# Daniel-Lin-S/decode_tonal_langauge

Hardware: AMD Instinct MI355X
Metric: mel-frames/sec (train step) SynthesisModelCNN, 128ch x 400t batch256 (higher is better)
Workload: dtype f32; 1 GPU; SynthesisModelCNN 128ch x 400t -> 80 mel, 4 tones x 2 syllables, L=5, global batch 256 (strong scaling: 256 windows on rank 0), dropout 0.5, NAdam, 1,376,768,720 params; per_gpu_batch=256, global_batch=256, parallelism=dp1, init=drawn on every rank

## Files before the change

### decode_tonal_langauge_amd/_conv_stack.py

```python
from __future__ import annotations

from typing import List

import torch

from . import _kernels, _lib
from ._launch import LaunchTimers, launch_nt, launch_tn, permute_reduce, r4
from ._lib import (EPI_C1WGRAD, EPI_GY, EPI_LRELU, EPI_MASK, EPI_MASKY, EPI_POOL, EPI_POOLV, LOAD_DIRECT, LOAD_UNPOOL, LOAD_V,
                   LOAD_Y, check, ptr)


class _Stage:

    def __init__(self, idx, cin, cout, k, pool, tin, tp_in):
        self.idx, self.cin, self.cout, self.k, self.pool = idx, cin, cout, k, pool
        self.tin, self.tp_in = tin, tp_in
        self.tc = tin - k + 1
        self.tout = self.tc // 2 if pool else self.tc
        self.tp_out = tp_in // 2 if pool else tp_in


class ConvStack(LaunchTimers):
    F63_CAPABLE = True

    def __init__(self, n_channels: int, n_timepoints: int, stage_defs, negative_slope: float, conv_channels: int):
        if negative_slope < 0:
            raise ValueError("the MI355X path needs negative_slope >= 0 (max-pool / LeakyReLU are fused)")
        self.lib = _lib.load()
        self.C = n_channels
        self.T = n_timepoints
        self.slope = float(negative_slope)
        k1 = stage_defs[0][1]
        npool_after = sum(1 for s in stage_defs[1:] if s[2])
        tc1 = n_timepoints - k1 + 1
        self.k1 = k1
        self.c1 = stage_defs[0][0]
        self.tout1 = tc1 // 2
        if not stage_defs[0][2]:
            raise ValueError("first stage must pool")
        align = 1 << npool_after
        self.tp1 = max(align, (self.tout1 + align - 1) // align * align)
        _kernels.validate()
        self.wino63 = (self.F63_CAPABLE and _kernels.get("wino") == "6"
                       and self._f63_covers(stage_defs, n_timepoints))
        tp1_default = self.tp1
        if self.wino63:
            self.tp1 = (self.tout1 + 11) // 12 * 12
        self.f63_yprod = (self.wino63 and _kernels.get("f63_yprod") != "0" and stage_defs[0][0] % 256 == 0
                          and self.tp1 >= 12)
        self.f63_yprod3 = (self.wino63 and _kernels.get("f63_yprod") != "0" and stage_defs[1][0] % 256 == 0)
        self.stages: List[_Stage] = []
        cin, tin, tp = self.c1, self.tout1, self.tp1
        for i, (cout, k, pool) in enumerate(stage_defs[1:], start=2):
            st = _Stage(i, cin, cout, k, pool, tin, tp)
            if st.tout < 1:
                raise ValueError("n_timepoints too small for the conv stack")
            if self.wino63 and i == 3:
                st.tp_out = tp1_default // 4
            self.stages.append(st)
            cin, tin, tp = cout, st.tout, st.tp_out
        self.gy4 = self._gy_applies()
        self.lat = tin
        self.tp5 = tp
        self.ld5 = r4(conv_channels)
        mode = _kernels.get("wino")
        self.wino43 = mode != "0"
        self.store_p1 = _kernels.get("store_p1") == "1"
        self.fuse_c1 = True
        self.wino_vout = True
        self.tn_bm = 0
        self._gy_A = None
        self._vhalo = {}
        self._B = None
        self.generation = 0

    def _alloc(self, B: int, dev) -> bool:
        if self._B == B and self._dev == dev:
            return False
        self._B, self._dev = B, dev
        self.S = B * self.C
        self._v_ready = {}
        self._gy_A = None
        self._vhalo = {}
        self._alloc_rows()
        self.Yt = {}
        self._y_ready = {}
        self.V = {}
        self.Vd = {}
        self._vd_ready = {}
        self.G = None
        return True

    def _alloc_rows(self):
        S, dev = self.S, self._dev
        z = lambda *s: torch.zeros(*s, dtype=torch.float32, device=dev)
        zi = lambda *s: torch.zeros(*s, dtype=torch.int32, device=dev)
        self.P = {}
        if not (self.wino63 or self._conv1_writes_v()) or self.store_p1:
            self.P[1] = z(S * self.tp1, self.c1)
        self.bits = {1: zi(S * self.tp1, self.c1 // 32)}
        self.sbits = {1: zi(S * self.tp1, self.c1 // 32)}
        for st in self.stages:
            rows = S * st.tp_out
            ld = st.cout if st.pool else self.ld5
            no_rows = (self.wino63 and st.idx == 2) or (self._writes_v(st) and not self._f63(st))
            if not no_rows or self.store_p1:
                self.P[st.idx] = z(rows, ld)
            if st.pool:
                self.bits[st.idx] = zi(rows, st.cout // 32)
                self.sbits[st.idx] = zi(rows, st.cout // 32)

    def _alloc_bwd(self) -> bool:
        if self.G is not None:
            return False
        z = lambda *s: torch.zeros(*s, dtype=torch.float32, device=self._dev)
        S = self.S
        self.G = {}
        if not self.wino63 and not (self.fuse_c1 and self._c1_fusable() and self._v43(self.stages[0])):
            self.G[1] = z(S * self.tp1, self.c1)
        for st in self.stages:
            if not (self.f63_yprod and st.idx == 2) and not (self.gy4 and st.idx == 3):
                self.G[st.idx] = z(S * st.tp_out, st.cout if st.pool else self.ld5)
        return True

    def _stream(self):
        return torch.cuda.current_stream().cuda_stream

    def _permute(self, src, dst, dims, strides, *args, **kw):
        permute_reduce(self.lib, src, dst, dims, strides, *args, **kw)

    def _nt(self, tag=None, fn="tl_gemm_nt_window", **kw):
        ev = self._tick(tag)
        launch_nt(self.lib, fn, **kw)
        if ev:
            ev[1].record()

    def _tn(self, tag=None, fn="tl_gemm_tn_window", **kw):
        ev = self._tick(tag)
        launch_tn(self.lib, fn, **kw)
        if ev:
            ev[1].record()

    @staticmethod
    def _splitk(tiles: int, ksteps: int, target: int = 2048) -> int:
        return int(max(1, min(ksteps, (target + tiles - 1) // tiles, 1024)))

    def _tn_stored(self, tag, At, ldt, W, rows, K):
        if ldt <= 32:
            sk = self._splitk((K + 511) // 512, (rows + 15) // 16, 1024)
        else:
            sk = self._splitk(((ldt + 127) // 128) * ((K + 127) // 128), (rows + 31) // 32, 1024)
        slab = torch.empty(sk, ldt, K, dtype=torch.float32, device=self._dev)
        self._tn(tag=tag, A=ptr(At), B=ptr(W), slab=ptr(slab), Krows=rows, A_rows=rows, B_rows=rows, Mdim=ldt, Ndim=K, lda=ldt,
                 ldb=K, ldc=K, loader=LOAD_DIRECT, splitk=sk, slab_stride=ldt * K)
        return slab, sk

    def _pack_conv(self, w, cin_ld, flip_for_dgrad):
        O, I, J, _ = w.shape
        if not flip_for_dgrad:
            dst = torch.empty(J, O, cin_ld, dtype=torch.float32, device=w.device)
            self._permute(w, dst, (1, J, O, cin_ld), (0, 1, I * J, J), (1, J, O, I))
            return dst
        old = r4(O)
        dst = torch.empty(J, cin_ld, old, dtype=torch.float32, device=w.device)
        self._permute(w, dst, (1, J, cin_ld, old), (0, -1, J, I * J), (1, J, I, O), src_off=J - 1)
        return dst

    @staticmethod
    def _f63_covers(stage_defs, T) -> bool:
        if len(stage_defs) < 4:
            return False
        (c1, k1, p1), (c2, k2, p2), (c3, k3, p3) = stage_defs[0], stage_defs[1], stage_defs[2]
        tout1 = (T - k1 + 1) // 2
        tout2 = (tout1 - 2) // 2
        tout3 = (tout2 - 2) // 2
        return (p1 and p2 and p3 and k2 == 3 and k3 == 3 and 1 <= k1 <= 3 and c1 in (128, 256, 512, 1024)
                and c2 % 128 == 0 and c3 % 64 == 0 and tout3 >= 1 and T >= 2 * tout1 + 2)

    def _f63(self, st) -> bool:
        return self.wino63 and st.idx in (2, 3)

    def _nt63_rows(self) -> int:
        return int(self.lib.tl_wino63_nt_tile_rows())

    def _v_hex_buffer(self, store, idx, rows, cin):
        nh = rows // 6
        nh_pad = (nh + 24 + 127) // 128 * 128
        V = store.get(idx)
        if V is None or V.shape[0] != nh_pad or V.shape[1] != 8 or V.shape[2] != cin:
            V = store[idx] = torch.zeros(nh_pad, 8, cin, dtype=torch.float32, device=self._dev)
        return V

    def _halo_buffer(self, key, ntm, cout):
        halo = self._vhalo.get(key)
        if halo is None or halo.shape[0] != ntm or halo.shape[2] != cout:
            halo = self._vhalo[key] = torch.zeros(ntm, 2, cout, dtype=torch.float32, device=self._dev)
        return halo

    def _pack_wino63(self, w, forward: bool):
        O, I = w.shape[0], w.shape[1]
        dst = torch.empty(8, O, I, dtype=torch.float32, device=w.device) if forward else \
            torch.empty(8, I, O, dtype=torch.float32, device=w.device)
        check(self.lib.tl_wino63_weights(ptr(w), ptr(dst) if forward else None, None if forward else ptr(dst), O, I, I, O,
                                         self._stream()), "tl_wino63_weights")
        return dst

    def f63_issue_factor(self, st) -> float:
        return (st.tp_in // 6) * 8.0 / (st.tc * 3.0)

    def _stage_forward63(self, st, w, bia) -> None:
        S = self.S
        wp = self._pack_wino63(w, True)
        V = self._v_ready[st.idx - 1]
        if st.idx == 2 and self.store_p1 and 2 not in self.P:
            self.P[2] = torch.zeros(S * st.tp_out, st.cout, dtype=torch.float32, device=self._dev)
        Pout = self.P.get(st.idx) if (st.idx != 2 or self.store_p1) else None
        kw = dict(A=ptr(V), A_rows=V.shape[0], lda=V.shape[2], loader=LOAD_V, Bw=ptr(wp), bias=ptr(bia), out=ptr(Pout),
                  M=S * st.tp_in, N=st.cout, K=st.cin, ldb=st.cin, ldo=Pout.shape[1] if Pout is not None else st.cout, J=3,
                  row_shift=0, Tp=st.tp_in, slope=self.slope, obits=ptr(self.bits[st.idx]), osign=ptr(self.sbits[st.idx]),
                  ld_obits=st.cout // 32, Tvalid=2 * st.tout)
        if st.idx == 2:
            rows_out = S * st.tp_out
            Vn = self._v_hex_buffer(self.V, 2, rows_out, st.cout)
            ntm = -(-(S * st.tp_in) // self._nt63_rows())
            halo = self._halo_buffer(2, ntm, st.cout)
            kw.update(epilogue=EPI_POOLV, vout=ptr(Vn), vhalo=ptr(halo), vout_quads=Vn.shape[0], ld_vout=Vn.shape[2])
            self._nt(tag="conv2_fwd", fn="tl_conv3_wino63v_nt", **kw)
            check(self.lib.tl_wino63_v_fixup(ptr(Vn), ptr(halo), rows_out // 6, ntm, st.tp_out, st.cout, Vn.shape[2],
                                             self._stream()), "tl_wino63_v_fixup")
            self._v_ready[2] = Vn
        else:
            if Pout is None:
                raise RuntimeError("F(6,3) stage 3 writes pooled rows: its output buffer was not allocated")
            kw.update(epilogue=EPI_POOL, out_tp=st.tp_out)
            self._nt(tag="conv3_fwd", fn="tl_conv3_wino63v_nt", **kw)

    def _stage_wgrad63(self, st, gw, gb) -> None:
        S = self.S
        f32 = dict(dtype=torch.float32, device=self._dev)
        rows_in = S * st.tp_in
        nd = st.cout
        ldg = nd
        V = self._v_ready[st.idx - 1]
        tiles = (st.cin // 64) * (nd // 64)
        sk = self._splitk(tiles, (rows_in + 35) // 36, 4096)
        slab = torch.empty(sk, 8 * st.cin, ldg, **f32)
        bias_part = torch.empty(sk, nd, **f32)
        if (st.idx == 3 and self.f63_yprod3 and self._y_ready.get(3) != self.generation):
            Gs = self.G[3]
            Y3 = self._v_hex_buffer(self.Yt, 3, rows_in, nd)
            Vd3 = self._v_hex_buffer(self.Vd, 3, rows_in, nd)
            ev = self._tick("conv3_yvd")
            check(self.lib.tl_wino63_unpool_yvd(ptr(Gs), ptr(self.bits[3]), ptr(Y3), ptr(Vd3), rows_in, Gs.shape[0], st.tp_in,
                                                st.tp_out, 2 * st.tout, nd, Gs.shape[1], st.cout // 32, nd, self._stream()),
                  "tl_wino63_unpool_yvd")
            if ev:
                ev[1].record()
            self._y_ready[3] = self.generation
            self._vd_ready[3] = self.generation
        if self._y_ready.get(st.idx) == self.generation:
            Y = self.Yt[st.idx]
            self._y_ready[st.idx] = -1
            self._tn(tag=f"conv{st.idx}_wgrad", fn="tl_conv3_wino63v_tn", A=ptr(V), B=ptr(Y), slab=ptr(slab), Krows=rows_in,
                     A_rows=V.shape[0], B_rows=Y.shape[0], Mdim=st.cin, Ndim=nd, lda=V.shape[2], ldb=Y.shape[2], ldc=ldg, J=3,
                     Tp=st.tp_in, splitk=sk, slab_stride=8 * st.cin * ldg, loader=LOAD_Y, Tvalid=2 * st.tout,
                     colsum=ptr(bias_part))
        else:
            Gs = self.G[st.idx]
            Vd = self._v_hex_buffer(self.Vd, st.idx, rows_in, nd)
            self._tn(tag=f"conv{st.idx}_wgrad", fn="tl_conv3_wino63v_tn", A=ptr(V), B=ptr(Gs), slab=ptr(slab), Krows=rows_in,
                     A_rows=V.shape[0], B_rows=Gs.shape[0], Mdim=st.cin, Ndim=nd, lda=V.shape[2], ldb=Gs.shape[1], ldc=ldg, J=3,
                     Tp=st.tp_in, splitk=sk, slab_stride=8 * st.cin * ldg, loader=LOAD_UNPOOL, bbits=ptr(self.bits[st.idx]),
                     ld_bbits=st.cout // 32, Tvalid=2 * st.tout, colsum=ptr(bias_part), vd=ptr(Vd), ld_vd=nd, g_tp=st.tp_out)
            self._vd_ready[st.idx] = self.generation
        self._wino_wgrad_tail(st, slab, bias_part, 8, "tl_wino63_wgrad_finalize", gw, gb)

    def _wino_wgrad_tail(self, st, slab, bias_part, taps, finalize, gw, gb) -> None:
        sk, rows, ldg = slab.shape
        if sk > 1:
            red = torch.empty(rows, ldg, dtype=torch.float32, device=self._dev)
            n = taps * st.cin * ldg
            self._permute(slab, red, (1, 1, 1, n), (0, 0, 0, 1), nz=sk, zs=n)
        else:
            red = slab
        check(getattr(self.lib, finalize)(ptr(red), ptr(gw), st.cout, st.cin, ldg, self._stream()), finalize)
        self._permute(bias_part, gb, (1, 1, 1, st.cout), (0, 0, 0, 1), nz=sk, zs=bias_part.shape[1])

    def _gy_stage(self, st) -> bool:
        return self.gy4 and st.idx == 4

    def _gy_applies(self) -> bool:
        if not (self.wino63 and self.f63_yprod3 and len(self.stages) >= 3):
            return False
        below, st = self.stages[1], self.stages[2]
        return (_kernels.get("conv4_dgrad") == "nt63" and st.k == 1 and st.pool and self._f63(below)
                and st.cout % 32 == 0 and st.cout >= 40 and st.cin % 32 == 0 and (below.tp_in // 2) % 3 == 0)

    def _stage_dgrad_gy(self, st, w):
        S = self.S
        below = self.stages[1]
        tpg = below.tp_in // 2
        rows = S * tpg
        f32 = dict(dtype=torch.float32, device=self._dev)
        nh = -(-rows // 6)
        nh_pad = (nh + 127) // 128 * 128
        A = self._gy_A
        if A is None or A.shape[0] != nh_pad or A.shape[2] != st.cout:
            A = self._gy_A = torch.zeros(nh_pad, 8, st.cout, **f32)
        Gs = self.G[st.idx]
        ev = self._tick(f"conv{st.idx}_dgrad")
        check(self.lib.tl_wino63_unpool_rows6(ptr(Gs), ptr(self.bits[st.idx]), ptr(A), rows, Gs.shape[0], tpg, st.tp_out,
                                              2 * st.tout, st.cout, Gs.shape[1], st.cout // 32, st.cout, 0, self._stream()),
              "tl_wino63_unpool_rows6")
        taps = torch.empty(st.cout // 8, 8, st.cin, 8, **f32)
        check(self.lib.tl_wino63_weights1(ptr(w), ptr(taps), st.cout, st.cin, st.cout, self._stream()), "tl_wino63_weights1")
        rows3 = S * below.tp_in
        Y3 = self._v_hex_buffer(self.Yt, below.idx, rows3, below.cout)
        Vd3 = self._v_hex_buffer(self.Vd, below.idx, rows3, below.cout)
        ntm = -(-rows // self._nt63_rows())
        halo = self._halo_buffer("d3", ntm, below.cout)
        self._nt(tag=None, fn="tl_conv1_wino63v_dgrad_nt", A=ptr(A), A_rows=A.shape[0], lda=A.shape[2], loader=LOAD_V,
                 Bw=ptr(taps), M=rows, N=st.cin, K=st.cout, ldb=st.cout, ldo=st.cin, J=1, row_shift=0, Tp=tpg, slope=self.slope,
                 auxbits=ptr(self.sbits[below.idx]), ld_auxbits=self.sbits[below.idx].shape[1], abits=ptr(self.bits[below.idx]),
                 ld_abits=below.cout // 32, out_tp=below.tp_out, Tvalid_in=2 * below.tout, epilogue=EPI_GY, out=None,
                 vout=ptr(Y3), vout2=ptr(Vd3), vhalo=ptr(halo), vout_quads=Y3.shape[0], ld_vout=Y3.shape[2])
        check(self.lib.tl_wino63_vd_fixup(ptr(Vd3), ptr(halo), rows // 3, ntm, below.tp_in // 6, below.cout, Vd3.shape[2],
                                          self._stream()), "tl_wino63_vd_fixup")
        if ev:
            ev[1].record()
        self._y_ready[below.idx] = self.generation
        self._vd_ready[below.idx] = self.generation
        return None

    def _stage_dgrad63(self, st, w):
        S = self.S
        rows_in = S * st.tp_in
        if self._vd_ready.get(st.idx) != self.generation:
            raise RuntimeError("F(6,3) input gradient: its operand (Vd from the stage's weight-gradient pass, or Y2 from the "
                               "input gradient of stage 3) must be written first")
        self._vd_ready[st.idx] = -1
        on_y = st.idx == 2 and self.f63_yprod
        Vd = self.Yt[2] if on_y else self.Vd[st.idx]
        if on_y:
            wd = torch.empty(8, st.cin, st.cout, dtype=torch.float32, device=w.device)
            check(self.lib.tl_wino63_weights_y(ptr(w), ptr(wd), st.cout, st.cin, st.cout, self._stream()), "tl_wino63_weights_y")
        else:
            wd = self._pack_wino63(w, False)
        kw = dict(A=ptr(Vd), A_rows=Vd.shape[0], lda=Vd.shape[2], loader=LOAD_V, Bw=ptr(wd), M=rows_in, N=st.cin,
                  K=st.cout, ldb=st.cout, ldo=st.cin, J=3, row_shift=0 if on_y else -2, Tp=st.tp_in, slope=self.slope,
                  auxbits=ptr(self.sbits[st.idx - 1]), ld_auxbits=self.sbits[st.idx - 1].shape[1])
        if st.idx == 3 and self.f63_yprod:
            below = self.stages[0]
            rows2 = S * below.tp_in
            Y2 = self._v_hex_buffer(self.Yt, 2, rows2, below.cout)
            Vd2 = self._v_hex_buffer(self.Vd, 2, rows2, below.cout) if self.store_p1 else None
            ntm = -(-rows_in // self._nt63_rows())
            halo = self._halo_buffer("d2", ntm, below.cout) if self.store_p1 else None
            self._nt(tag="conv3_dgrad", fn="tl_conv3_wino63v_nt", epilogue=EPI_MASKY, out=None, vout=ptr(Y2), vout2=ptr(Vd2),
                     vhalo=ptr(halo), vout_quads=Y2.shape[0], ld_vout=Y2.shape[2], abits=ptr(self.bits[2]),
                     ld_abits=below.cout // 32, Tvalid_in=2 * below.tout, **kw)
            if Vd2 is not None:
                check(self.lib.tl_wino63_vd_fixup(ptr(Vd2), ptr(halo), rows_in // 3, ntm, below.tp_in // 6, below.cout,
                                                  Vd2.shape[2], self._stream()), "tl_wino63_vd_fixup")
            self._y_ready[2] = self.generation
            self._vd_ready[2] = self.generation
            return None
        if st.idx == 3:
            self._nt(tag="conv3_dgrad", fn="tl_conv3_wino63v_nt", epilogue=EPI_MASK, out=ptr(self.G[2]), **kw)
            return None
        ntm = -(-rows_in // self._nt63_rows())
        part = torch.empty(ntm, (self.k1 + 1) * self.c1, dtype=torch.float32, device=self._dev)
        self._nt(tag="conv2_dgrad", fn="tl_conv3_wino63v_nt", epilogue=EPI_C1WGRAD, out=None, c1x=ptr(self._x),
                 c1bits=ptr(self.bits[1]), c1partial=ptr(part), c1T=self.T, c1kt=self.k1, Tvalid=self.tout1, **kw)
        return part

    def _c1_fusable(self) -> bool:
        return self.k1 <= 3 and self.T >= 2 * self.tout1 + 2

    def _v43(self, st) -> bool:
        return (self.wino43 and st.k == 3 and st.pool and st.cin % 64 == 0 and st.cout % 32 == 0 and st.tp_in % 4 == 0
                and r4(st.cout) % 16 == 0)

    def _tn_bm(self, st) -> int:
        wide = st.cin % 128 == 0
        dma8 = wide and r4(st.cout) % 64 == 0 and (st.cout // 32) % 2 == 0
        if self.tn_bm == 127:
            return 127 if wide else 64
        if self.tn_bm in (0, 128):
            return 128 if dma8 else 64
        return 64

    def _conv1_writes_v(self) -> bool:
        return (self._v43(self.stages[0]) and self.tp1 % 4 == 0 and self.c1 in (128, 256, 512, 1024)
                and (self.fuse_c1 and self._c1_fusable()))

    def _writes_v(self, st) -> bool:
        if not (self.wino_vout and st.pool and st.idx - 1 < len(self.stages)):
            return False
        nxt = self.stages[st.idx - 1]
        return self._v43(st) and self._v43(nxt) and st.tp_in % 8 == 0 and nxt.cin == st.cout

    def _pin(self, st):
        return self.P.get(st.idx - 1)

    def _v_buffer(self, idx, rows, cin, store=None):
        store = self.V if store is None else store
        nq = rows // 4
        nq_pad = (nq + 127) // 128 * 128
        V = store.get(idx)
        if V is None or V.shape[0] != nq_pad or V.shape[2] != cin:
            V = store[idx] = torch.zeros(nq_pad, 6, cin, dtype=torch.float32, device=self._dev)
        return V

    def _input_transform(self, st):
        src = self.P[st.idx - 1]
        V = self._v_buffer(st.idx - 1, src.shape[0], st.cin)
        ev = self._tick(f"conv{st.idx}_xform")
        check(self.lib.tl_wino43_input_transform(ptr(src), ptr(V), src.shape[0], st.tp_in, st.cin, src.shape[1], st.cin,
                                                 self._stream()), "tl_wino43_input_transform")
        if ev:
            ev[1].record()
        return V

    def wgrad_issue_factor(self, st) -> float:
        if self._f63(st):
            return self.f63_issue_factor(st)
        return 0.5 if self._v43(st) else 1.0

    def kernel_families(self):
        if self.wino63:
            self._fam_share = {}
            st2, st3 = self.stages[0], self.stages[1]
            f6 = "Winograd F(6,3) on pre-transformed operands, LDS-DMA"
            tn = "wino63v_tn4_kernel<true>" if st3.cin % 256 == 0 and st3.tp_in >= 12 else "wino63v_tn_kernel<true>"
            tn2 = "wino63v_tn4_kernel<true>" if st2.cin % 256 == 0 else "wino63v_tn_kernel<true>"
            fams = {f"wino63v_nt_kernel<POOLV> (conv2 forward, {f6}; writes V of its pooled output for conv3)": ["conv2_fwd"],
                    f"wino63v_nt_kernel<POOL> (conv3 forward, {f6})": ["conv3_fwd"],
                    f"wino63v_nt_kernel<C1WGRAD> (conv2 input gradient + conv1 weight gradient, {f6})": ["conv2_dgrad"],
                    }
            if self.f63_yprod3:
                gy = self.gy4
                src = "the epilogue of conv4's input gradient" if gy else "wino63_unpool_yvd_kernel"
                fams[f"wino63v_tn4y_kernel (conv3 weight gradient, {f6}: both operands by LDS-DMA, no transform in the kernel; Y3 / Vd3 "
                     f"from {src})"] = ["conv3_wgrad"]
            else:
                fams[f"{tn} (conv3 weight gradient, {f6}; also writes Vd)"] = ["conv3_wgrad"]
            if self.f63_yprod:
                both = "Y and Vd" if self.store_p1 else "Y"
                fams[f"wino63v_nt_kernel<MASKY> (conv3 input gradient, {f6}; writes {both} of conv2 instead of the gradient rows)"] = ["conv3_dgrad"]
                fams[f"wino63v_tn4y_kernel (conv2 weight gradient, {f6}: both operands by LDS-DMA, no transform in the kernel)"] = ["conv2_wgrad"]
            else:
                fams[f"wino63v_nt_kernel<MASK> (conv3 input gradient, {f6})"] = ["conv3_dgrad"]
                fams[f"{tn2} (conv2 weight gradient, {f6}; also writes Vd)"] = ["conv2_wgrad"]
            issued = {k: self.f63_issue_factor(st2 if "conv2" in k else st3) for k in fams}
            return fams, issued
        self._fam_share = {}
        if not all(self._v43(st) for st in self.stages[:2]):
            fams = {"nt_window_kernel<128,UNPOOL,MASK> (conv input-gradient)": ["conv2_dgrad", "conv3_dgrad", "conv4_dgrad"],
                    "nt_window_kernel<128,DIRECT,POOL> (conv forward)": ["conv2_fwd", "conv3_fwd", "conv4_fwd"],
                    "tn3_kernel<UNPOOL> (conv weight-gradient)": ["conv2_wgrad", "conv3_wgrad"]}
            return fams, {k: 1.0 for k in fams}
        form = "Winograd F(4,3) on pre-transformed operands, LDS-DMA"
        fused = self.fuse_c1 and self._c1_fusable()
        bm = self._tn_bm(self.stages[0])
        extra = {}
        if bm == 128:
            tn = f"wino43v_tn8_kernel<true> (conv2/conv3 weight gradient, {form}; also writes Vd for the input gradient)"
        else:
            ntm = (self.stages[0].cin + 63) // 64
            tn = f"wino43v_tn_kernel<false, 2> (conv2/conv3 weight gradient, C_in tiles 1..{ntm - 1} of {ntm}, {form})"
            vdn = f"wino43v_tn_kernel<true, 2> (conv2/conv3 weight gradient, C_in tile 0 of {ntm}, {form}, + writes Vd for the input gradient)"
            extra[vdn] = ["conv2_wgrad_vd", "conv3_wgrad_vd"]
            self._fam_share = {tn: (ntm - 1) / ntm, vdn: 1.0 / ntm}
        fams = {tn: ["conv2_wgrad", "conv3_wgrad"]}
        if self._writes_v(self.stages[0]):
            fams[f"wino43v_nt_kernel<POOLV> (conv2 forward, {form}; writes V of its pooled output for conv3 instead of the raw rows)"] = ["conv2_fwd"]
            fams[f"wino43v_nt_kernel<POOL> (conv3 forward, {form})"] = ["conv3_fwd"]
        else:
            fams[f"wino43v_nt_kernel<POOL> (conv2/conv3 forward, {form})"] = ["conv2_fwd", "conv3_fwd"]
        fams.update(extra)
        if fused:
            fams[f"wino43v_nt_kernel<UNPOOL,C1WGRAD> (conv2 input gradient + conv1 weight gradient, {form})"] = ["conv2_dgrad"]
            fams[f"wino43v_nt_kernel<UNPOOL,MASK> (conv3 input gradient, {form})"] = ["conv3_dgrad"]
        else:
            fams[f"wino43v_nt_kernel<UNPOOL,MASK> (conv2/conv3 input gradient, {form})"] = ["conv2_dgrad", "conv3_dgrad"]
        return fams, {k: 0.5 for k in fams}

    def _pack_wino43(self, w, forward: bool):
        O, I = w.shape[0], w.shape[1]
        dst = torch.empty(6, O, I, dtype=torch.float32, device=w.device) if forward else \
            torch.empty(6, I, O, dtype=torch.float32, device=w.device)
        check(self.lib.tl_wino43_weights(ptr(w), ptr(dst) if forward else None, None if forward else ptr(dst), O, I, I, O,
                                         self._stream()), "tl_wino43_weights")
        return dst

    def conv1_forward(self, x, w1, b1) -> None:
        lib, st_ = self.lib, self._stream()
        S, T, dev = self.S, self.T, self._dev
        self._x = x
        self._v_ready = {}
        w1 = w1.reshape(self.c1, self.k1).contiguous()
        sbits = ptr(self.sbits.get(1))
        if self.store_p1 and 1 not in self.P:
            self.P[1] = torch.zeros(S * self.tp1, self.c1, dtype=torch.float32, device=dev)
        P1 = ptr(self.P[1]) if self.store_p1 else None
        geom = (S, T, self.k1, self.c1, self.tp1, self.tout1, self.slope, st_)
        if self.wino63:
            V1 = self._v_hex_buffer(self.V, 1, S * self.tp1, self.c1)
            ev = self._tick("conv1_fwd")
            check(lib.tl_conv1_fwd_v6(ptr(x), ptr(w1), ptr(b1), P1, ptr(V1), ptr(self.bits[1]), sbits, *geom), "tl_conv1_fwd_v6")
            if ev:
                ev[1].record()
            self._v_ready[1] = V1
        elif self._conv1_writes_v():
            V1 = self._v_buffer(1, S * self.tp1, self.c1)
            check(lib.tl_conv1_fwd_v(ptr(x), ptr(w1), ptr(b1), P1, ptr(V1), ptr(self.bits[1]), sbits, *geom), "tl_conv1_fwd_v")
            self._v_ready[1] = V1
        else:
            check(lib.tl_conv1_fwd(ptr(x), ptr(w1), ptr(b1), ptr(self.P[1]), ptr(self.bits[1]), sbits, *geom), "tl_conv1_fwd")

    STAGE_NAMES = {2: "ecog_conv_block.3", 3: "ecog_conv_block.6", 4: "ecog_conv_block.9", 5: "ecog_conv_block.12"}

    def stage_forward(self, st: _Stage, w: torch.Tensor, bia: torch.Tensor) -> None:
        if self._f63(st):
            return self._stage_forward63(st, w, bia)
        S = self.S
        v43 = self._v43(st)
        wp = self._pack_wino43(w, True) if v43 else self._pack_conv(w, st.cin, False)
        src = self._pin(st)
        vout = self._writes_v(st)
        if vout and self.store_p1 and st.idx not in self.P:
            self.P[st.idx] = torch.zeros(S * st.tp_out, st.cout, dtype=torch.float32, device=self._dev)
        Pout = self.P.get(st.idx) if (not vout or self.store_p1) else None
        kw = dict(A=ptr(src), Bw=ptr(wp), bias=ptr(bia), out=ptr(Pout), M=S * st.tp_in,
                  A_rows=S * st.tp_in, N=st.cout, K=st.cin, lda=st.cin, ldb=st.cin,
                  ldo=Pout.shape[1] if Pout is not None else st.cout, J=st.k, row_shift=0, Tp=st.tp_in, slope=self.slope,
                  loader=LOAD_DIRECT)
        if st.pool:
            kw.update(epilogue=EPI_POOL, obits=ptr(self.bits[st.idx]), osign=ptr(self.sbits[st.idx]),
                      ld_obits=st.cout // 32, Tvalid=2 * st.tout)
        else:
            kw.update(epilogue=EPI_LRELU, Tvalid=st.tout)
        if not v43:
            self._nt(tag=f"conv{st.idx}_fwd", fn="tl_gemm_nt_window", **kw)
            return
        V = self._v_ready.get(st.idx - 1)
        if V is None:
            V = self._v_ready[st.idx - 1] = self._input_transform(st)
        kw.update(A=ptr(V), A_rows=V.shape[0], lda=V.shape[2], loader=LOAD_V)
        if vout:
            rows_out = S * st.tp_out
            Vn = self._v_buffer(st.idx, rows_out, st.cout)
            ntm = (S * st.tp_in + 511) // 512
            halo = self._halo_buffer(st.idx, ntm, st.cout)
            kw.update(epilogue=EPI_POOLV, vout=ptr(Vn), vhalo=ptr(halo), vout_quads=Vn.shape[0], ld_vout=Vn.shape[2])
            self._nt(tag=f"conv{st.idx}_fwd", fn="tl_conv3_wino43v_nt", **kw)
            check(self.lib.tl_wino43_v_fixup(ptr(Vn), ptr(halo), rows_out // 4, ntm, st.tp_out, st.cout, Vn.shape[2],
                                             self._stream()), "tl_wino43_v_fixup")
            self._v_ready[st.idx] = Vn
            return
        self._nt(tag=f"conv{st.idx}_fwd", fn="tl_conv3_wino43v_nt", **kw)

    def _colsum(self, Gm, rows, ncols, ld, Tp, Tvalid, dst):
        nc4 = r4(ncols)
        rpb = max(1, 256 // (nc4 // 4))
        nblk = int(min(2048, max(1, rows // (rpb * 16))))
        part = torch.empty(nblk, nc4, dtype=torch.float32, device=Gm.device)
        check(self.lib.tl_colsum(ptr(Gm), ptr(part), nblk, rows, nc4, ld, Tp, Tvalid, self._stream()), "tl_colsum")
        self._permute(part, dst, (1, 1, 1, ncols), (0, 0, 0, 1), nz=nblk, zs=nc4)

    def _reduce_c1_partials(self, part: torch.Tensor, gw: torch.Tensor, gb: torch.Tensor) -> None:
        f32 = dict(dtype=torch.float32, device=part.device)
        nblk = part.shape[0]
        zs = (self.k1 + 1) * self.c1
        if nblk >= 256 and zs % 4 == 0:
            red = torch.empty(zs, **f32)
            flat = part.view(-1)
            for c0 in range(0, zs, 1024):
                nc = min(1024, zs - c0)
                self._colsum(flat[c0:], nblk, nc, zs, 1, 1, red[c0:c0 + nc])
            self._permute(red, gw, (1, 1, self.c1, self.k1), (0, 0, 1, self.c1))
            self._permute(red, gb, (1, 1, 1, self.c1), (0, 0, 0, 1), src_off=self.k1 * self.c1)
        else:
            self._permute(part, gw, (1, 1, self.c1, self.k1), (0, 0, 1, self.c1), nz=nblk, zs=zs)
            self._permute(part, gb, (1, 1, 1, self.c1), (0, 0, 0, 1), nz=nblk, zs=zs, src_off=self.k1 * self.c1)

    def stage_wgrad(self, st: _Stage, gw: torch.Tensor, gb: torch.Tensor) -> None:
        if self._f63(st):
            return self._stage_wgrad63(st, gw, gb)
        S = self.S
        f32 = dict(dtype=torch.float32, device=self._dev)
        Xin = self._pin(st)
        Gs = self.G[st.idx]
        rows_in = S * st.tp_in
        ldg = Gs.shape[1]
        nd = r4(st.cout)
        if self._v43(st):
            tiles = ((st.cin + 63) // 64) * ((nd + 63) // 64)
            bm = self._tn_bm(st)
            sk = self._splitk(tiles, (rows_in + 31) // 32, 4096 if bm in (127, 128) else 8192)
            slab = torch.empty(sk, 6 * st.cin, ldg, **f32)
            bias_part = torch.empty(sk, nd, **f32)
# ... 87 lines not shown
```

### decode_tonal_langauge_amd/_kernels.py

```python
from __future__ import annotations

import os
from typing import Callable, Dict, Tuple, Union

_Allowed = Union[frozenset, Callable[[str], bool]]


def _int(lo: int, hi: int) -> Callable[[str], bool]:
    def ok(v: str) -> bool:
        try:
            return lo <= int(v) <= hi
        except ValueError:
            return False
    return ok


_B = frozenset({"0", "1"})
KEYS: Dict[str, Tuple[str, _Allowed, str, str]] = {
    "wino": ("TONAL_WINO", frozenset({"6", "4", "0"}), "6",
             "conv2 / conv3: 6 Winograd F(6,3) on pre-transformed operands (F(4,3) V form where the stack does not allow it), "
             "4 the F(4,3) V form, 0 direct MFMA kernels (also the fallback for every shape neither form covers)"),
    "f63_yprod": ("TONAL_F63_YPROD", _B, "1", "F(6,3): the backward operands of stages 2 and 3 (Y2 for both passes of stage 2; Y3 / Vd3) come "
                                              "pre-transformed out of the input-gradient epilogue of the stage above (0: the weight-gradient "
                                              "kernels un-pool and transform the gradient rows themselves and write Vd)"),
    "conv4_dgrad": ("TONAL_CONV4_DGRAD", frozenset({"nt63", "gemm"}), "nt63",
                    "F(6,3): the one-tap stage behind conv3 - nt63: its input gradient on the NT63 kernel, writing Y3 / Vd3 "
                    "(no gradient rows, no tl_wino63_unpool_yvd); gemm: one-tap GEMM + tl_wino63_unpool_yvd"),
    "store_p1": ("TONAL_STORE_P1", _B, "0", "keep the raw pooled rows of stages 1 / 2 beside V, and Vd2 beside Y2 (tests)"),
    "conv7": ("TONAL_CONV7", frozenset({"wino63", "wino63bwd", "direct"}), "wino63",
              "the CNN-RNN classifier's 7-tap convolutions: wino63 three F(6,3) segments forward, direct kernels backward; "
              "wino63bwd the same forward and, in training, both backward passes on F(6,3) as well; direct all direct"),
    "whh_dh": ("TONAL_WHH_DH", _B, "1", "single process: the W_hh NAdam pass also produces the last BPTT product dh_1 = dgates_2 . W_hh "
                                        "(0: a W_hh stream of its own for it)"),
    "whh_stream": ("TONAL_WHH_STREAM", _B, "1", "label LSTM backward: dgates . W_hh as a pure stream of the weight (tl_lstm_gw; 0: the skinny "
                                                "MFMA GEMM with split-K slabs, also the form for more than 8 distinct label rows)"),
    "graph": ("TONAL_GRAPH", _B, "1", "SynthesisLite step replayed as a HIP graph"),
    "lstm_shard": ("TONAL_LSTM_SHARD", _B, "1", "data parallel: label LSTM sharded by gate rows"),
    "hilbert": ("TONAL_HILBERT", frozenset({"auto", "ols", "ols_full", "sym", "taps", "fft"}), "auto",
                "Hilbert bank: force a path (ols band-limited overlap-save, ols_full all 1024 bins per band, sym / taps the "
                "time-domain kernels with / without Hermitian symmetry, fft the DFT-domain form)"),
    "hilbert_f32": ("TONAL_HILBERT_F32", _B, "0", "float32 recordings: fp32 transforms end to end (default: fp64 math)"),
    "butter": ("TONAL_BUTTER", frozenset({"seq", "scan"}), "seq",
               "zero-phase Butterworth: seq the sequential recurrence (bit-identical to scipy's loop), scan the time-parallel "
               "block scan (2e-8 - 5e-8 from it: the size of the reference's own rounding; ~20 x faster)"),
}
_LEGACY = {v[0]: k for k, v in KEYS.items()}
_cache: Tuple[str, Dict[str, str]] = ("", {})


def _check(key: str, value: str) -> str:
    allowed = KEYS[key][1]
    ok = allowed(value) if callable(allowed) else value in allowed
    if not ok:
        what = "an integer in range" if callable(allowed) else "one of " + ", ".join(sorted(allowed))
        raise ValueError(f"TONAL_KERNELS: {key}={value!r} is not a value this switch takes ({what})")
    return value


def _parsed() -> Dict[str, str]:
    global _cache
    raw = os.environ.get("TONAL_KERNELS", "")
    if raw == _cache[0]:
        return _cache[1]
    out: Dict[str, str] = {}
    for item in raw.split(","):
        item = item.strip()
        if not item:
            continue
        key, sep, value = item.partition("=")
        key, value = key.strip(), value.strip()
        if not sep or key not in KEYS:
            raise ValueError(f"TONAL_KERNELS: unknown setting {item!r}; keys: " + ", ".join(sorted(KEYS)))
        out[key] = _check(key, value)
    _cache = (raw, out)
    return out


def get(key: str, default: str = None) -> str:
    legacy, _allowed, table_default, _doc = KEYS[key]
    spec = _parsed()
    if key in spec:
        return spec[key]
    if legacy in os.environ:
        if os.environ.get("TONAL_AB") != "1":
            raise RuntimeError(f"{legacy} is an A/B switch of the test suite and is ignored by the product: use "
                               f"TONAL_KERNELS={key}={os.environ[legacy]} (or set TONAL_AB=1 to run an A/B comparison)")
        return _check(key, os.environ[legacy])
    return table_default if default is None else default


def conv7_forward() -> str:
    form = get("conv7")
    return "wino63" if form == "wino63bwd" else form


def validate() -> None:
    _parsed()
    if os.environ.get("TONAL_AB") != "1":
        for legacy, key in _LEGACY.items():
            if legacy in os.environ:
                get(key)
```

### decode_tonal_langauge_amd/csrc/tonal_wino63.hip

```cpp
#include "tonal_common.h"
#include "tonal_wino43_epi.h"
#include "tonal_wino43v_epi.h"
#include "tonal_wino63_epi.h"
#include "tonal_wino63_kloop.h"
#include <type_traits>

namespace tl {

typedef __attribute__((address_space(3))) void lds_void6_t;
__device__ __forceinline__ void dma16h(__amdgpu_buffer_rsrc_t rs, char* lds_dst, unsigned voff, unsigned soff) {
  __builtin_amdgcn_raw_ptr_buffer_load_lds(rs, (lds_void6_t*)lds_dst, 16, voff, soff, 0, 0);
}

typedef int v6_i32x4 __attribute__((ext_vector_type(4)));
__device__ __forceinline__ v6_i32x4 v6_rsrc_words(const void* base, long long bytes) {
  const unsigned long long a = (unsigned long long)base;
  const long long n = bytes < 0 ? 0 : (bytes < 0x7fffffffLL ? bytes : 0x7fffffffLL);
  return v6_i32x4{(int)(unsigned)a, (int)(unsigned)((a >> 32) & 0xffffu), (int)n, 0x00020000};
}

__device__ __forceinline__ long long v6_at(long long hex, int i, int c, int kc8) {
  return ((((hex >> 1) * kc8 + (c >> 3)) * 8 + i) * 2 + (hex & 1)) * 8 + (c & 7);
}

// ... 48 lines not shown
  for (int t = 0; t < 8; ++t) m[t] = s[t * plane];
  const float a12 = m[1] + m[2], s12 = m[1] - m[2], a34 = m[3] + m[4], s34 = m[3] - m[4], a56 = m[5] + m[6], s56 = m[5] - m[6];
  float* d = gw + ((long long)o * I + i) * 3;
  d[0] = -m[0] - (2.f / 9.f) * a12 + (1.f / 90.f) * a34 + (32.f / 45.f) * a56;
  d[1] = -(2.f / 9.f) * s12 + (1.f / 45.f) * s34 + (16.f / 45.f) * s56;
  d[2] = -(2.f / 9.f) * a12 + (2.f / 45.f) * a34 + (8.f / 45.f) * a56 + m[7];
}

__global__ void wino63_weights7_kernel(const float* __restrict__ w, float* __restrict__ fwd, int O, int I, int taps) {
  const long long idx = (long long)blockIdx.x * blockDim.x + threadIdx.x;
  if (idx >= 3LL * O * I) return;
  const int k = (int)(idx % (3LL * I)), o = (int)(idx / (3LL * I));
  const int seg = k / I, i = k - seg * I;
  const float* s = w + ((long long)o * I + i) * taps + 3 * seg;
  const float g0 = 3 * seg < taps ? s[0] : 0.f, g1 = 3 * seg + 1 < taps ? s[1] : 0.f, g2 = 3 * seg + 2 < taps ? s[2] : 0.f;
  float* d0 = fwd + (((long long)(k >> 3) * 8) * O + o) * 8 + (k & 7);
  const long long n = (long long)O * 8;
  const float sm = g0 + g2;
  d0[0] = -g0;
  d0[n] = (-2.f / 9.f) * (sm + g1);
  d0[2 * n] = (-2.f / 9.f) * (sm - g1);
  const float a = fmaf(4.f, g2, g0), b = 2.f * g1;
  d0[3 * n] = (1.f / 90.f) * (a + b);
  d0[4 * n] = (1.f / 90.f) * (a - b);
  const float c = fmaf(4.f, g0, g2), d = 2.f * g1;
  d0[5 * n] = (8.f / 45.f) * (c + d);
  d0[6 * n] = (8.f / 45.f) * (c - d);
  d0[7 * n] = g2;
}

__global__ __launch_bounds__(256, 4) void wino63_xform2_kernel(const float* __restrict__ P, float* __restrict__ V0, float* __restrict__ V1,
                                                             long long nhex, int hps, int Tp, int Tvalid, int C, int ldp, int ldv,
                                                             int shift) {
  const int tpp = C >> 1;
  const long long idx = (long long)blockIdx.x * blockDim.x + threadIdx.x;
  const long long pair = idx / tpp;
  const int tl_ = (int)(idx - pair * tpp);
  const int half = tl_ & 1, hpar = (tl_ >> 1) & 1, kc = tl_ >> 2;
  const int c = 8 * kc + 4 * half;
  const long long hg = 2 * pair + hpar;
  if (hg >= nhex) return;
  const long long seq = hg / hps;
  const int hs = (int)(hg - seq * hps);
  const float* src = P + (seq * Tp + 6LL * hs) * (long long)ldp + c;
  f32x4 d[11];
#pragma unroll
  for (int j = 0; j < 11; ++j) {
    d[j] = f32x4{0.f, 0.f, 0.f, 0.f};
    const int t = 6 * hs + j - shift;
    if (t >= 0 && t < Tvalid) d[j] = *reinterpret_cast<const f32x4*>(src + (long long)(j - shift) * ldp);
  }
  f32x4 o0[8], o1[8];
#pragma unroll
  for (int k = 0; k < 4; ++k) {
    float a[8], b[8], va[8], vb[8];
#pragma unroll
    for (int j = 0; j < 8; ++j) {
      a[j] = d[j][k];
      b[j] = d[j + 3][k];
    }
    wino63_bt(a, va);
    wino63_bt(b, vb);
#pragma unroll
    for (int j = 0; j < 8; ++j) {
      o0[j][k] = va[j];
      o1[j][k] = vb[j];
    }
  }
  const long long at = v6_at(hg, 0, c, ldv >> 3);
#pragma unroll
  for (int j = 0; j < 8; ++j) *reinterpret_cast<f32x4*>(V0 + at + 16 * j) = o0[j];
#pragma unroll
  for (int j = 0; j < 8; ++j) *reinterpret_cast<f32x4*>(V1 + at + 16 * j) = o1[j];
}

__global__ __launch_bounds__(256, 4) void wino63_ydz_kernel(const float* __restrict__ G, float* __restrict__ Y, long long nhex, int hps,
                                                          int Tp, int Tvalid, int C, int ldg, int ldv) {
  const int tpp = C >> 1;
  const long long idx = (long long)blockIdx.x * blockDim.x + threadIdx.x;
  const long long pair = idx / tpp;
  const int tl_ = (int)(idx - pair * tpp);
  const int half = tl_ & 1, hpar = (tl_ >> 1) & 1, kc = tl_ >> 2;
  const int c = 8 * kc + 4 * half;
  const long long hg = 2 * pair + hpar;
  if (hg >= nhex) return;
  const long long seq = hg / hps;
  const int hs = (int)(hg - seq * hps);
  const float* src = G + (seq * Tp + 6LL * hs) * (long long)ldg + c;
  f32x4 d[6];
#pragma unroll
  for (int j = 0; j < 6; ++j) {
    d[j] = f32x4{0.f, 0.f, 0.f, 0.f};
    if (6 * hs + j < Tvalid) d[j] = *reinterpret_cast<const f32x4*>(src + (long long)j * ldg);
  }
  f32x4 oy[8];
#pragma unroll
  for (int k = 0; k < 4; ++k) {
    const float d6[6] = {d[0][k], d[1][k], d[2][k], d[3][k], d[4][k], d[5][k]};
    const float ev1 = (d6[0] + d6[2]) + d6[4], od1 = (d6[1] + d6[3]) + d6[5];
    const float ev2 = fmaf(16.f, d6[4], fmaf(4.f, d6[2], d6[0])), od2 = fmaf(32.f, d6[5], fmaf(8.f, d6[3], 2.f * d6[1]));
    const float ev3 = fmaf(0.0625f, d6[4], fmaf(0.25f, d6[2], d6[0])), od3 = fmaf(0.03125f, d6[5], fmaf(0.125f, d6[3], 0.5f * d6[1]));
    const float y[8] = {d6[0], ev1 + od1, ev1 - od1, ev2 + od2, ev2 - od2, ev3 + od3, ev3 - od3, d6[5]};
#pragma unroll
    for (int j = 0; j < 8; ++j) oy[j][k] = y[j];
  }
  const long long at = v6_at(hg, 0, c, ldv >> 3);
#pragma unroll
  for (int j = 0; j < 8; ++j) *reinterpret_cast<f32x4*>(Y + at + 16 * j) = oy[j];
}

__global__ __launch_bounds__(256, 4) void wino63_v_fixup_kernel(float* __restrict__ V, const float* __restrict__ halo, long long hexes,
                                                              long long tiles, int Tq, int C, int ldv) {
  const int c4n = C >> 2;
  const long long idx = (long long)blockIdx.x * blockDim.x + threadIdx.x;
  if (idx >= tiles * c4n) return;
  const long long t = idx / c4n;
  const int c = (int)(idx - t * c4n) * 4;
  const long long q = t * 64 + 63;
  if (q >= hexes) return;
  float* v = V + v6_at(q, 0, c, ldv >> 3);
  f32x4 d[8];
#pragma unroll
  for (int j = 0; j < 6; ++j) d[j] = *reinterpret_cast<const f32x4*>(v + 16 * j);
  const int tq = (int)((6 * q) % Tq);
  if (tq + 6 < Tq && t + 1 < tiles) {
    d[6] = *reinterpret_cast<const f32x4*>(halo + ((t + 1) * 2) * (long long)C + c);
    d[7] = *reinterpret_cast<const f32x4*>(halo + ((t + 1) * 2 + 1) * (long long)C + c);
  } else {
    d[6] = d[7] = f32x4{0.f, 0.f, 0.f, 0.f};
  }
  f32x4 o[8];
#pragma unroll
  for (int k = 0; k < 4; ++k) {
    float dd[8], vv[8];
#pragma unroll
    for (int j = 0; j < 8; ++j) dd[j] = d[j][k];
    wino63_bt(dd, vv);
#pragma unroll
    for (int j = 0; j < 8; ++j) o[j][k] = vv[j];
  }
#pragma unroll
  for (int j = 0; j < 8; ++j) *reinterpret_cast<f32x4*>(v + 16 * j) = o[j];
}

constexpr int V6_BH = 128, V6_BN = 64, V6_BK = 8;
constexpr int V6_ROWB = V6_BK * 4;
constexpr int V6_A_BYTES = 8 * V6_BH * V6_ROWB;
constexpr int V6_B_BYTES = 8 * V6_BN * V6_ROWB;
constexpr int V6_STAGE = V6_A_BYTES + V6_B_BYTES;
constexpr int V6_ROWS = 6 * V6_BH;

template <int EPI>
__global__ __launch_bounds__(512, 2) void wino63v_nt_kernel(const tl_nt_params p) {
  __shared__ __attribute__((aligned(1024))) char lds[3 * V6_STAGE + ((EPI == W_EPI_POOLV || EPI == W_EPI_MASKY || EPI == W_EPI_GY) ? 4096 : (EPI == W_EPI_C1W || EPI == W6_EPI_C1W_Y) ? 16384 : 0)];
  const int tid = threadIdx.x;
  const int lane = tid & 63;
  const int wave = __builtin_amdgcn_readfirstlane(tid >> 6);
  const int wm = wave >> 1, wn = wave & 1;
  const int lr = lane & 31, lh = lane >> 5;

  const int ntn = (p.N + V6_BN - 1) / V6_BN;
  const long long ntm = (p.M + V6_ROWS - 1) / V6_ROWS;
  const long long nwg = ntm * ntn;
  constexpr bool SEG3 = EPI == W_EPI_LRELU || EPI == W6_EPI_MASK7 || EPI == W6_EPI_MASK7F;
  constexpr bool SIX = EPI == W_EPI_GY;
  const int kseg = p.K / V6_BK;
  const int nsteps = SEG3 ? 3 * kseg : kseg;
  f32x16 acc[8];
  f32x4 faL[4], fbL[4], faH[4], fbH[4];

  const int prow = lane >> 1;
  const int src_chunk = (lane & 1) ^ ((lane >> 4) & 1);
  const v6_i32x4 rsB = v6_rsrc_words(p.Bw, (SIX && wave >= 6) ? 0 : 8LL * p.N * p.ldb * 4);
  const unsigned lds0 = (unsigned)(unsigned long long)(lds_void6_t*)lds;
  const unsigned dst_a0 = lds0 + (unsigned)(wave * V6_BH * V6_ROWB);
  const unsigned dst_b0 = lds0 + (unsigned)(V6_A_BYTES + wave * V6_BN * V6_ROWB);
  const int hex_of_row = (prow & 3) | ((prow >> 3) << 2) | (((prow >> 2) & 1) << 4);
  const int kc8 = p.lda >> 3;
  unsigned avoff[4], bv_lane[2];
#pragma unroll
  for (int t = 0; t < 4; ++t) avoff[t] = (unsigned)(v6_at(t * 32 + hex_of_row, wave, src_chunk * 4, kc8) * 4);
  unsigned avoff1[4];
#pragma unroll
  for (int t = 0; t < 4; ++t) avoff1[t] = SEG3 ? (unsigned)(v6_at(t * 32 + hex_of_row + 1, wave, src_chunk * 4, kc8) * 4) : avoff[t];
#pragma unroll
  for (int t = 0; t < 2; ++t) bv_lane[t] = (unsigned)((((long long)wave * p.N + t * 32 + prow) * 8 + src_chunk * 4) * 4);
  const unsigned b_step = (unsigned)p.N * 256u;

  struct tile_t {
    long long tm, R0;
    int n0;
    v6_i32x4 rsA, rsA1;
    unsigned bvoff[2];
  };
  const long long a_tile_bytes = (long long)V6_BH * 8 * p.lda * 4, a_total_bytes = p.A_rows * 8LL * p.lda * 4;
  auto place = [&](tile_t& t, long long tm, int tn) {
    t.tm = tm;
    t.R0 = tm * V6_ROWS;
    t.n0 = tn * V6_BN;
    const long long ab = tm * a_tile_bytes;
    t.rsA = v6_rsrc_words(reinterpret_cast<const char*>(p.A) + ab, (SIX && wave >= 6) ? 0 : a_total_bytes - ab);
    t.rsA1 = SEG3 ? v6_rsrc_words(reinterpret_cast<const char*>(p.aux) + ab, a_total_bytes - ab) : t.rsA;
    if (t.n0 + V6_BN <= p.N) {
      const unsigned nb4 = (unsigned)t.n0 * 32u;
#pragma unroll
      for (int k = 0; k < 2; ++k) t.bvoff[k] = bv_lane[k] + nb4;
    } else {
#pragma unroll
      for (int k = 0; k < 2; ++k) {
        int n = t.n0 + k * 32 + prow;
        if (n > p.N - 1) n = p.N - 1;
        t.bvoff[k] = (unsigned)((((long long)wave * p.N + n) * 8 + src_chunk * 4) * 4);
      }
    }
  };
  tile_t cur;
  {
    long long bid = blockIdx.x;
    const long long q = nwg / 8, r = nwg % 8, x = bid % 8, i = bid / 8;
    bid = (x < r ? x * (q + 1) : r * (q + 1) + (x - r) * q) + i;
    place(cur, bid / ntn, (int)(bid % ntn));
  }
  const int walk = (int)(gridDim.x >> 3), walk_q = walk / ntn, walk_r = walk - walk_q * ntn;
  auto advance = [&](const tile_t& c) -> tile_t {
    tile_t t = c;
    int tn = c.n0 / V6_BN + walk_r;
    long long tm = c.tm + walk_q;
    if (tn >= ntn) {
      tn -= ntn;
      ++tm;
    }
    place(t, tm, tn);
    return t;
  };
  auto next3 = [](int s) { return s == 2 ? 0 : s + 1; };

  const int cphys = (lh ^ ((lr >> 3) & 1)) << 4;
  const unsigned a_row = lds0 + (unsigned)((wm * 32 + lr) * V6_ROWB + cphys);
  const unsigned b_row = lds0 + (unsigned)((wn * 32 + lr) * V6_ROWB + cphys);
  int stg = 0;

  struct dma_src {
    v6_i32x4 ra;
    unsigned va[4], vb[2], sa, sb;
  };
  auto src_of = [&](const tile_t& t, int step) {
    dma_src d;
    int ks = step;
    if constexpr (SEG3) {
      const int seg = (step >= kseg ? 1 : 0) + (step >= 2 * kseg ? 1 : 0);
      ks = step - seg * kseg;
#pragma unroll
      for (int k = 0; k < 4; ++k) {
        d.ra[k] = seg == 1 ? t.rsA1[k] : t.rsA[k];
        d.va[k] = seg == 2 ? avoff1[k] : avoff[k];
      }
    } else {
      d.ra = t.rsA;
#pragma unroll
      for (int k = 0; k < 4; ++k) d.va[k] = avoff[k];
    }
    d.vb[0] = t.bvoff[0];
    d.vb[1] = t.bvoff[1];
#pragma unroll
    for (int k = 0; k < 4; ++k) d.ra[k] = __builtin_amdgcn_readfirstlane(d.ra[k]);
    d.sa = (unsigned)__builtin_amdgcn_readfirstlane(ks * 512);
    d.sb = (unsigned)__builtin_amdgcn_readfirstlane((int)((unsigned)step * b_step));
    return d;
  };
#define V6K_INPUTS(src, dst, wimm)                                                                                             \
  [a] "v"(a_row + (unsigned)stg * (unsigned)V6_STAGE), [b] "v"(b_row + (unsigned)stg * (unsigned)V6_STAGE),                    \
      [va0] "v"((src).va[0]), [va1] "v"((src).va[1]), [va2] "v"((src).va[2]), [va3] "v"((src).va[3]), [vb0] "v"((src).vb[0]), \
      [vb1] "v"((src).vb[1]), [ra] "s"((src).ra), [rb] "s"(rsB), [m0a] "s"(dst_a0 + (unsigned)(dst) * (unsigned)V6_STAGE),     \
      [m0b] "s"(dst_b0 + (unsigned)(dst) * (unsigned)V6_STAGE), [sa] "s"((src).sa), [sb] "s"((src).sb), [w] "n"(wimm)
#pragma clang diagnostic ignored "-Winline-asm"
#define V6K_STMT_R(REGS, TEXT, tl_, step, dst, wimm)                                                                     \
  do {                                                                                                                   \
    const dma_src src_ = src_of(tl_, step);                                                                              \
    asm volatile(TEXT : REGS(acc, faL, fbL, faH, fbH) : V6K_INPUTS(src_, dst, wimm) : "memory", "scc", "m0");                  \
  } while (0)
#define V6K_STMT(TEXT, tl_, step, dst, wimm) V6K_STMT_R(V6K_REGS, TEXT, tl_, step, dst, wimm)
  auto issue = [&](const tile_t& tl_, int step, int dst) {
    const dma_src src_ = src_of(tl_, step);
    asm volatile(V6K_ISSUE : : V6K_INPUTS(src_, dst, 0) : "memory", "scc", "m0");
  };
  constexpr bool early = EPI == W_EPI_POOLV || EPI == W_EPI_C1W || EPI == W6_EPI_C1W_Y;
  constexpr int NST = v6_stores<EPI>();
  constexpr int first_n = NST + 6 > 63 ? 63 : NST + 6;
  constexpr int first_wait = (first_n & 15) | (7 << 4) | (0 << 8) | ((first_n >> 4) << 14);

  issue(cur, 0, 0);
  issue(cur, 1, 1);
  __builtin_amdgcn_s_waitcnt(0x0f70);
  for (long long vb = blockIdx.x; vb < nwg; vb += gridDim.x) {
    __builtin_amdgcn_s_barrier();
    asm volatile("" ::: "memory");
    auto prefetch = [&] {
      if constexpr (EPI == W_EPI_POOL || EPI == W_EPI_POOLV || EPI == W_EPI_LRELU) return v5_prefetch_pool(p, cur.n0, wn, lr);
      else if constexpr (EPI == W_EPI_MASK || EPI == W6_EPI_MASK7) return v6_prefetch_mask(p, cur.R0, cur.n0, wm, wn, lr, lh);
      else if constexpr (EPI == W6_EPI_MASK7F) return v6_pre_mask{{0u, 0u, 0u}};
      else if constexpr (EPI == W_EPI_MASKY || EPI == W6_EPI_MASKY_Y) return v6_prefetch_masky(p, cur.R0, cur.n0, wm, wn, lr, lh);
      else if constexpr (EPI == W_EPI_GY) return v6_prefetch_masky<true>(p, cur.R0, cur.n0, wm, wn, lr, lh);
      else return v6_prefetch_c1w(p, cur.R0, cur.n0, wm, wn, lr, lh);
    };
    decltype(prefetch()) pre;
#define V6K_RUN(KIND, RSFX, tl_, step, dst, wimm)                                                                              \
  do {                                                                                                                         \
    if constexpr (SIX) V6K_STMT_R(V6K6_REGS##RSFX, V6K6_##KIND##_L, tl_, step, dst, wimm);                                     \
    else if constexpr (early) V6K_STMT_R(V6K_REGS##RSFX, V6K_##KIND##_E, tl_, step, dst, wimm);                                \
    else V6K_STMT_R(V6K_REGS##RSFX, V6K_##KIND##_L, tl_, step, dst, wimm);                                                     \
  } while (0)
    if constexpr (SIX) V6K_STMT_R(V6K6_REGS_FIRST, V6K6_FIRST, cur, 2, stg == 0 ? 2 : stg - 1, first_wait);
    else V6K_STMT_R(V6K_REGS_FIRST, V6K_FIRST, cur, 2, stg == 0 ? 2 : stg - 1, first_wait);
    stg = next3(stg);
    V6K_RUN(STEP1, _STEP1, cur, 3, stg == 0 ? 2 : stg - 1, 0);
    stg = next3(stg);
    {
      int s = 2;
      do {
        V6K_RUN(NORM, , cur, s + 2, stg == 0 ? 2 : stg - 1, 0);
        stg = next3(stg);
      } while (++s + 2 < nsteps);
    }
    V6K_RUN(PRELAST, , cur, 0, 0, 0);
    stg = next3(stg);
    pre = prefetch();
    V6K_RUN(LAST, , cur, 0, 0, 0);
    stg = next3(stg);
#undef V6K_RUN

    const tile_t done = cur;
    const long long nb = vb + gridDim.x;
    const int last_stage = stg == 0 ? 2 : stg - 1;
    __builtin_amdgcn_s_waitcnt(0x0f70);
    if (nb < nwg) {
      cur = advance(cur);
      issue(cur, 0, stg);
      issue(cur, 1, next3(stg));
    }
    __builtin_amdgcn_sched_barrier(0);
    float* scratch = reinterpret_cast<float*>(lds + last_stage * V6_STAGE);
    (void)scratch;
    const bool full = done.R0 + V6_ROWS <= p.M && done.n0 + V6_BN <= p.N;
    if constexpr (EPI == W_EPI_POOL) {
      if (full) v6_epilogue_pool<false, true>(p, acc, pre, nullptr, done.R0, done.n0, wm, wn, lr, lh, done.tm);
      else v6_epilogue_pool<false, false>(p, acc, pre, nullptr, done.R0, done.n0, wm, wn, lr, lh, done.tm);
    } else if constexpr (EPI == W_EPI_POOLV) {
      float* xch = reinterpret_cast<float*>(lds + 3 * V6_STAGE);
      if (full) v6_epilogue_pool<true, true>(p, acc, pre, xch, done.R0, done.n0, wm, wn, lr, lh, done.tm);
      else v6_epilogue_pool<true, false>(p, acc, pre, xch, done.R0, done.n0, wm, wn, lr, lh, done.tm);
    } else if constexpr (EPI == W_EPI_LRELU) {
      if (full) v6_epilogue_lrelu<true>(p, acc, pre, done.R0, done.n0, wm, wn, lr, lh);
      else v6_epilogue_lrelu<false>(p, acc, pre, done.R0, done.n0, wm, wn, lr, lh);
    } else if constexpr (EPI == W_EPI_MASK || EPI == W6_EPI_MASK7) {
      if (full) v6_epilogue_mask<true>(p, acc, pre, done.R0, done.n0, wm, wn, lr, lh);
      else v6_epilogue_mask<false>(p, acc, pre, done.R0, done.n0, wm, wn, lr, lh);
    } else if constexpr (EPI == W6_EPI_MASK7F) {
      if (full) v6_epilogue_mask<true, true>(p, acc, pre, done.R0, done.n0, wm, wn, lr, lh);
      else v6_epilogue_mask<false, true>(p, acc, pre, done.R0, done.n0, wm, wn, lr, lh);
    } else if constexpr (EPI == W_EPI_MASKY) {
      float* xch = reinterpret_cast<float*>(lds + 3 * V6_STAGE);
      if (full) v6_epilogue_masky<true>(p, acc, pre, xch, done.R0, done.n0, wm, wn, lr, lh, done.tm);
      else v6_epilogue_masky<false>(p, acc, pre, xch, done.R0, done.n0, wm, wn, lr, lh, done.tm);
    } else if constexpr (EPI == W6_EPI_MASKY_Y) {
      if (full) v6_epilogue_masky<true, false, false>(p, acc, pre, nullptr, done.R0, done.n0, wm, wn, lr, lh, done.tm);
      else v6_epilogue_masky<false, false, false>(p, acc, pre, nullptr, done.R0, done.n0, wm, wn, lr, lh, done.tm);
    } else if constexpr (EPI == W_EPI_GY) {
      float* xch = reinterpret_cast<float*>(lds + 3 * V6_STAGE);
      if (full) v6_epilogue_masky<true, true>(p, acc, pre, xch, done.R0, done.n0, wm, wn, lr, lh, done.tm);
      else v6_epilogue_masky<false, true>(p, acc, pre, xch, done.R0, done.n0, wm, wn, lr, lh, done.tm);
    } else {
      v6_epilogue_c1w<EPI == W6_EPI_C1W_Y>(p, acc, pre, reinterpret_cast<float*>(lds + 3 * V6_STAGE) + wave * 512, scratch, done.R0,
                                           done.n0, wm, wn, lr, lh, done.tm);
    }
    {
      constexpr int n = NST + 6 > 63 ? 63 : NST + 6;
      __builtin_amdgcn_s_waitcnt((n & 15) | (7 << 4) | (15 << 8) | ((n >> 4) << 14));
    }
  }
}



constexpr int T6_BN = 64, T6_H = 6;
constexpr int T6_PLANE = T6_H * 64;
constexpr int T6_TILE = 8 * T6_PLANE;
constexpr int T6_NA = 4, T6_NG = 6;
constexpr int T6_GW = T6_H * 4 * 64;
constexpr int T6_GT = T6_GW + 64;

template <bool WVD>
__global__ __launch_bounds__(512, 1) void wino63v_tn_kernel(const tl_tn_params p, int mtn) {
  constexpr int NA = T6_NA, NG = T6_NG, GW = T6_GW, GT = T6_GT;
  __shared__ __attribute__((aligned(1024))) float lds[(NA * 2 + 2) * T6_TILE + NG * GT];
  float* As = lds;
  float* Bs = lds + NA * 2 * T6_TILE;
  float* Gs = Bs + 2 * T6_TILE;
  const int tid = threadIdx.x, lane = tid & 63;
  const int wave = __builtin_amdgcn_readfirstlane(tid >> 6);
  const int wm = wave >> 1, wn = wave & 1, lr = lane & 31, lh = lane >> 5;
  const int ntn = p.Ndim / T6_BN;
  const long long tiles = (long long)mtn * ntn;
  const long long nwg = tiles * p.splitk;
  long long bid = (long long)blockIdx.y * gridDim.x + blockIdx.x;
  {
    const long long q = nwg / 8, r = nwg % 8, x = bid % 8, i = bid / 8;
    bid = (x < r ? x * (q + 1) : r * (q + 1) + (x - r) * q) + i;
  }
  const int z = __builtin_amdgcn_readfirstlane((int)(bid / tiles));
  const int tt = __builtin_amdgcn_readfirstlane((int)(bid % tiles));
  const int mi = __builtin_amdgcn_readfirstlane(tt / ntn);
  const int m0 = mi * 128, n0 = __builtin_amdgcn_readfirstlane((tt % ntn) * T6_BN);

  const long long hexes_all = p.Krows / 6;
  const long long ksteps_all = (hexes_all + T6_H - 1) / T6_H;
  const long long per = __builtin_amdgcn_readfirstlane((int)((ksteps_all + p.splitk - 1) / p.splitk));
  const long long ks_begin = z * per;
  long long ks_end = ks_begin + per;
  if (ks_end > ksteps_all) ks_end = ksteps_all;
  const int nsteps = ks_end > ks_begin ? (int)(ks_end - ks_begin) : 0;

  f32x16 acc[8];
#pragma unroll
  for (int i = 0; i < 8; ++i)
#pragma unroll
    for (int e = 0; e < 16; ++e) acc[i][e] = 0.f;

  const long long v_h0 = ks_begin * T6_H;
  const int kc8 = p.lda >> 3;
  const __amdgpu_buffer_rsrc_t rsV = __builtin_amdgcn_make_buffer_rsrc(
      (void*)(p.A + v_h0 * 8 * (long long)p.lda), 0, clip31((p.A_rows - v_h0) * 8 * (long long)p.lda * 4), 0x00020000);
  unsigned vvoff[3], vdst[3];
#pragma unroll
  for (int t = 0; t < 3; ++t) {
    const int half = (wave * 3 + t) / 12, pc = (wave * 3 + t) % 12;
    const int rho = 4 * pc + (lane >> 4), i = rho / 6, hx = rho % 6;
    const int chunk = (lane & 15) ^ ((hx & 1) << 3);
    vvoff[t] = (unsigned)(v6_at(hx, i, m0 + half * 64 + chunk * 4, kc8) * 4);
    vdst[t] = (unsigned)((half * T6_TILE + pc * 256) * 4);
  }
  const unsigned v_step = (unsigned)(T6_H * 8 * p.lda * 4);
  auto issue_v = [&](int step) {
    char* base = reinterpret_cast<char*>(As) + (step & (NA - 1)) * (2 * T6_TILE * 4);
    const unsigned soff = (unsigned)step * v_step;
#pragma unroll
    for (int t = 0; t < 3; ++t) dma16h(rsV, base + vdst[t], vvoff[t] + soff, 0u);
  };
  const int Tq = p.Tp >> 1, hps = p.Tp / 6;
  const int g_tp = p.g_tp > 0 ? p.g_tp : Tq;
  const bool wpiece = wave >= 6;
  const int myhex = wpiece ? (lane >> 3) : wave;
  const long long seq0 = v_h0 / hps;
  const int hs0 = (int)(v_h0 - seq0 * hps);
  const long long g_r0 = seq0 * g_tp + 3LL * hs0;
  int g_hs = hs0 + myhex, g_off = 3 * myhex;
  while (g_hs >= hps) {
    g_hs -= hps;
    g_off += g_tp - Tq;
  }
  const int ldw4 = p.ld_bbits * 4;
  const __amdgpu_buffer_rsrc_t rsG = __builtin_amdgcn_make_buffer_rsrc(
      wpiece ? (void*)(p.bbits + g_r0 * (long long)p.ld_bbits + (n0 >> 5)) : (void*)(p.B + g_r0 * (long long)p.ldb + n0), 0,
      wpiece ? clip31((p.B_rows - g_r0) * (long long)ldw4 - (long long)(n0 >> 5) * 4)
             : clip31((p.B_rows - g_r0) * (long long)p.ldb * 4 - (long long)n0 * 4),
      0x00020000);
  const unsigned g_lane = wpiece ? (unsigned)(((lane >> 1) & 3) * ldw4 + (lane & 1) * 4)
                                 : (unsigned)(((lane >> 4) * (long long)p.ldb + (lane & 15) * 4) * 4);
  const unsigned g_row4 = wpiece ? (unsigned)ldw4 : (unsigned)(p.ldb * 4);
  const unsigned gdst = wpiece ? (unsigned)(GW * 4) : (unsigned)(wave * 256 * 4);
  const bool g_live = !wpiece || lane < 48;
  auto issue_g = [&](int slot) {
    const unsigned voff = g_live ? (unsigned)g_off * g_row4 + g_lane : 0xfffffff0u;
    if (wpiece) __builtin_amdgcn_raw_ptr_buffer_load_lds(rsG, (lds_void6_t*)(reinterpret_cast<char*>(Gs) + slot * (GT * 4) + gdst), 4, voff, 0u, 0, 0);
    else dma16h(rsG, reinterpret_cast<char*>(Gs) + slot * (GT * 4) + gdst, voff, 0u);
    g_hs += T6_H;
    g_off += 3 * T6_H;
    while (g_hs >= hps) {
      g_hs -= hps;
      g_off += g_tp - Tq;
    }
  };
  auto next6 = [](int v) { return v == NG - 1 ? 0 : v + 1; };

  constexpr bool write_vd = WVD;
  const bool ywave = wave < T6_H;
  const int sw = lane ^ ((wave & 1) << 5);
  int tq = __builtin_amdgcn_readfirstlane((int)((6 * (v_h0 + (ywave ? wave : 0))) % p.Tp));
  const int dstep = __builtin_amdgcn_readfirstlane((6 * T6_H) % p.Tp);
  float bsum = 0.f;
  const int kcd = write_vd ? (p.ld_vd >> 3) : 1;
  const unsigned vd_pstride = (unsigned)(16 * p.ld_vd * 4);
  const long long vd_hexes = ((hexes_all + 1) >> 1) << 1;
  const __amdgpu_buffer_rsrc_t rsVd = __builtin_amdgcn_make_buffer_rsrc(
      write_vd ? (void*)(p.vd + v_h0 * 8 * (long long)p.ld_vd) : (void*)p.slab, 0,
      write_vd ? clip31((vd_hexes - v_h0) * 8 * (long long)p.ld_vd * 4) : 0, 0x00020000);
  const unsigned vdA_lane = (unsigned)(v6_at(0, lane & 3, n0 + (lane & ~3), kcd) * 4);
  const unsigned vdB_lane = vdA_lane + 4u * 64u;
  const int nhex = (int)hexes_all, h_first = (int)v_h0;
  const int h_end = h_first + nsteps * T6_H;
  const int hs_lim = nhex < h_end ? nhex : h_end;
  struct y_in {
    float g[3];
    unsigned long long mo[3], me[3];
    int tq;
  };
  struct y_out {
    float d[6];
  };
  auto uni = [](unsigned long long v) -> unsigned long long {
    return (unsigned long long)(unsigned)__builtin_amdgcn_readfirstlane((int)(unsigned)v) |
           ((unsigned long long)(unsigned)__builtin_amdgcn_readfirstlane((int)(unsigned)(v >> 32)) << 32);
  };
  const int wy = ywave ? wave : 0;
  auto fetch_y = [&](int sd, int slot, y_in& y) {
    const int h = h_first + sd * T6_H + wy;
    const int live = ywave & (h < hs_lim);
    const float* gs = Gs + slot * GT;
    const unsigned long long* ws = reinterpret_cast<const unsigned long long*>(gs + GW) + wy * 4;
#pragma unroll
    for (int r = 0; r < 3; ++r) {
      y.g[r] = gs[wy * 256 + r * 64 + lane];
      const unsigned long long w = uni(ws[r]);
      const int v = live & (tq + 2 * r < p.Tvalid);
// ... 444 lines not shown
  };
#pragma unroll
  for (int i = 0; i < 8; ++i) fac[i] = 0.f;
#pragma unroll
  for (int i = 0; i < 4; ++i) fbc[i] = 0.f;

  {
    issue_v(0);
    issue_v(1);
    issue_v(2);
    issue_g(0);
    issue_g(1);
    issue_g(2);
    issue_g(3);
    float gp0 = 0.f;
    unsigned long long wp0 = 0ull;
    if (write_vd && hs0 > 0) {
      const long long pr = g_r0 - 1;
      if (pr < p.B_rows) {
        gp0 = p.B[pr * (long long)p.ldb + n0 + lane];
        const uint32_t* wsrc = p.bbits + pr * (long long)p.ld_bbits + (n0 >> 5);
        wp0 = (unsigned long long)wsrc[0] | ((unsigned long long)wsrc[1] << 32);
      }
    }
    __builtin_amdgcn_s_waitcnt(0x0070);
    __builtin_amdgcn_s_barrier();
    asm volatile("" ::: "memory");
    {
      y_in y0;
      fetch_y(0, 0, y0);
      const y_out u0 = compute_y(0, y0);
      if (write_vd && mi == 0) {
        float gp;
        unsigned long long wp;
        front_row(0, NG - 1, gp, wp);
        if (wave == 0) {
          gp = gp0;
          wp = uni(wp0);
        }
        vd_part(0, y0.tq, u0, gp, wp);
      }
    }
    __builtin_amdgcn_s_waitcnt(0x0070);
    __builtin_amdgcn_s_barrier();
    asm volatile("" ::: "memory");
  }
  int slot1 = 1, slot4 = 4;
  int turn = 1;
  for (int s = 0; s < nsteps; ++s) {
    const int abuf = s & (NA - 1), bbuf = s & 1;
    const int slot0 = slot1 == 0 ? NG - 1 : slot1 - 1;
    __builtin_amdgcn_sched_barrier(0);
    issue_v(s + 3);
    issue_g(slot4);
    y_raw yr;
    fetch_raw(slot1, yr);
    load_frag(fa0, fb0, abuf, bbuf, 0);
    mfma8(fac, fbc);
    load_frag(fa1, fb1, abuf, bbuf, 1);
    mfma8(fa0, fb0);
    __builtin_amdgcn_sched_group_barrier(0x100, 6 + 6, 0);
#pragma unroll
    for (int t = 0; t < 16; ++t) {
      __builtin_amdgcn_sched_group_barrier(0x008, 1, 0);
      if (t < 4) __builtin_amdgcn_sched_group_barrier(0x010, 1, 0);
      if (t >= 4 && t < 10) __builtin_amdgcn_sched_group_barrier(0x100, 1, 0);
    }
    __builtin_amdgcn_sched_barrier(0);
    load_frag(fac, fbc, abuf, bbuf, 2);
    y_in yn;
    y_out un = {};
    masks_y(s + 1, yr, yn);
    un = compute_y(s + 1, yn);
    mfma8(fa1, fb1);
    __builtin_amdgcn_sched_group_barrier(0x100, 6, 0);
#pragma unroll
    for (int t = 0; t < 8; ++t) {
      __builtin_amdgcn_sched_group_barrier(0x008, 1, 0);
      __builtin_amdgcn_sched_group_barrier(0x002, 5, 0);
      if (t >= 6) __builtin_amdgcn_sched_group_barrier(0x200, 2, 0);
    }
    __builtin_amdgcn_sched_barrier(0);
    if constexpr (write_vd) {
      if (ywave && turn == mi && s + 1 < nsteps) {
        float gp;
        unsigned long long wp;
        front_row(slot1, slot0, gp, wp);
        vd_part(s + 1, yn.tq, un, gp, wp);
      }
      turn = turn + 1 == nslots ? 0 : turn + 1;
    }
    __builtin_amdgcn_s_waitcnt(0x0078);
    __builtin_amdgcn_s_barrier();
    asm volatile("" ::: "memory");
    slot1 = next6(slot1);
    slot4 = next6(slot4);
  }
  mfma8(fac, fbc);

  if (p.colsum != nullptr && mi == 0) {
    __syncthreads();
    float* red = lds;
    red[wave * 64 + lane] = ywave ? bsum : 0.f;
    __syncthreads();
    if (tid < 64) {
      float t = 0.f;
#pragma unroll
      for (int q = 0; q < T6_H; ++q) t += red[q * 64 + tid];
      p.colsum[(long long)z * p.Ndim + n0 + tid] = t;
    }
  }
  float* out = p.slab + (long long)z * p.slab_stride;
  const int col = n0 + wn * 32 + lr;
#pragma unroll
  for (int i = 0; i < 8; ++i)
#pragma unroll
    for (int e = 0; e < 16; ++e) {
      const int m = m0 + wm * 64 + (i >> 2) * 32 + (e & 3) + 8 * (e >> 2) + 4 * lh;
      out[((long long)(i0 + (i & 3)) * p.Mdim + m) * (long long)p.ldc + col] = acc[i][e];
    }
}

__global__ __launch_bounds__(256, 4) void wino63_vd_fixup_kernel(float* __restrict__ Vd, const float* __restrict__ halo, long long hexes,
                                                               long long tiles, int hps, int C, int ldv) {
  const int c4n = C >> 2;
  const long long idx = (long long)blockIdx.x * blockDim.x + threadIdx.x;
  if (idx >= tiles * c4n) return;
  const long long t = idx / c4n;
  const int c = (int)(idx - t * c4n) * 4;
  const long long q = t * 256;
  if (q >= hexes) return;
  float* v = Vd + v6_at(q, 0, c, ldv >> 3);
  f32x4 d[8];
#pragma unroll
  for (int j = 2; j < 8; ++j) d[j] = *reinterpret_cast<const f32x4*>(v + 16 * j);
  if (t > 0 && (q % hps) != 0) {
    d[0] = *reinterpret_cast<const f32x4*>(halo + ((t - 1) * 2) * (long long)C + c);
    d[1] = *reinterpret_cast<const f32x4*>(halo + ((t - 1) * 2 + 1) * (long long)C + c);
  } else {
    d[0] = d[1] = f32x4{0.f, 0.f, 0.f, 0.f};
  }
  f32x4 o[8];
#pragma unroll
  for (int k = 0; k < 4; ++k) {
    float dd[8], vv[8];
#pragma unroll
    for (int j = 0; j < 8; ++j) dd[j] = d[j][k];
    wino63_bt(dd, vv);
#pragma unroll
    for (int j = 0; j < 8; ++j) o[j][k] = vv[j];
  }
#pragma unroll
  for (int j = 0; j < 8; ++j) *reinterpret_cast<f32x4*>(v + 16 * j) = o[j];
}

__global__ __launch_bounds__(512, 1) void wino63v_tn4y_kernel(const tl_tn_params p, int mtn) {
  constexpr int NA = 4;
  constexpr int QT = 4 * T6_PLANE;
  __shared__ __attribute__((aligned(1024))) float lds[NA * 4 * QT + NA * QT + 256];
  float* As = lds;
  float* Ys = lds + NA * 4 * QT;
  const int tid = threadIdx.x, lane = tid & 63;
  const int wave = __builtin_amdgcn_readfirstlane(tid >> 6);
  const int wm = wave >> 1, wn = wave & 1, lr = lane & 31, lh = lane >> 5;
  const int ntn = p.Ndim / T6_BN;
  const long long tiles = 2LL * mtn * ntn;
  const long long nwg = tiles * p.splitk;
  long long bid = (long long)blockIdx.y * gridDim.x + blockIdx.x;
  {
    const long long q = nwg / 8, r = nwg % 8, x = bid % 8, i = bid / 8;
    bid = (x < r ? x * (q + 1) : r * (q + 1) + (x - r) * q) + i;
  }
  const int z = __builtin_amdgcn_readfirstlane((int)(bid / tiles));
  const int tt = __builtin_amdgcn_readfirstlane((int)(bid % tiles));
  const int mi = __builtin_amdgcn_readfirstlane(tt % (2 * mtn));
  const int th = mi & 1, i0 = 4 * th;
  const int m0 = (mi >> 1) * 256, n0 = __builtin_amdgcn_readfirstlane((tt / (2 * mtn)) * T6_BN);
  const long long hexes_all = p.Krows / 6;
  const long long ksteps_all = (hexes_all + T6_H - 1) / T6_H;
  const long long per = __builtin_amdgcn_readfirstlane((int)((ksteps_all + p.splitk - 1) / p.splitk));
  const long long ks_begin = z * per;
  long long ks_end = ks_begin + per;
  if (ks_end > ksteps_all) ks_end = ksteps_all;
  const int nsteps = ks_end > ks_begin ? (int)(ks_end - ks_begin) : 0;

  f32x16 acc[8];
#pragma unroll
  for (int i = 0; i < 8; ++i)
#pragma unroll
    for (int e = 0; e < 16; ++e) acc[i][e] = 0.f;

  const long long v_h0 = ks_begin * T6_H;
  const int kc8 = p.lda >> 3, kcy = p.ldb >> 3;
  const __amdgpu_buffer_rsrc_t rsV = __builtin_amdgcn_make_buffer_rsrc(
      (void*)(p.A + v_h0 * 8 * (long long)p.lda), 0, clip31((p.A_rows - v_h0) * 8 * (long long)p.lda * 4), 0x00020000);
  const __amdgpu_buffer_rsrc_t rsY = __builtin_amdgcn_make_buffer_rsrc(
      (void*)(p.B + v_h0 * 8 * (long long)p.ldb), 0, clip31((p.B_rows - v_h0) * 8 * (long long)p.ldb * 4), 0x00020000);
  unsigned vvoff[3], vdst[3];
#pragma unroll
  for (int t = 0; t < 3; ++t) {
    const int quarter = (wave * 3 + t) / 6, pc = (wave * 3 + t) % 6;
    const int rho = 4 * pc + (lane >> 4), i = rho / 6, hx = rho % 6;
    const int chunk = (lane & 15) ^ ((hx & 1) << 3);
    vvoff[t] = (unsigned)(v6_at(hx + p.a_hex, i0 + i, m0 + quarter * 64 + chunk * 4, kc8) * 4);
    vdst[t] = (unsigned)((quarter * QT + pc * 256) * 4);
  }
  const bool ypiece = wave < T6_H;
  unsigned yvoff;
  {
    const int rho = 4 * (ypiece ? wave : 0) + (lane >> 4), i = rho / 6, hx = rho % 6;
    const int chunk = (lane & 15) ^ ((hx & 1) << 3);
    yvoff = (unsigned)(v6_at(hx, i0 + i, n0 + chunk * 4, kcy) * 4);
  }
  const unsigned v_step = (unsigned)(T6_H * 8 * p.lda * 4), y_step = (unsigned)(T6_H * 8 * p.ldb * 4);
  auto issue = [&](int step) {
    char* vb = reinterpret_cast<char*>(As) + (step & (NA - 1)) * (4 * QT * 4);
    const unsigned soff = (unsigned)step * v_step;
#pragma unroll
    for (int t = 0; t < 3; ++t) dma16h(rsV, vb + vdst[t], vvoff[t] + soff, 0u);
    char* yb = reinterpret_cast<char*>(Ys) + (ypiece ? ((step & (NA - 1)) * QT + wave * 256) * 4 : NA * QT * 4);
    dma16h(rsY, yb, ypiece ? yvoff + (unsigned)step * y_step : 0xfffffff0u, 0u);
  };
  const int a_off0 = wm * QT + lh * 64 + (lr ^ (lh << 5)), a_off1 = wm * QT + lh * 64 + ((32 + lr) ^ (lh << 5));
  const int b_off = lh * 64 + ((wn * 32 + lr) ^ (lh << 5));
  float fa0[8], fb0[4], fa1[8], fb1[4], fac[8], fbc[4];
  auto load_frag = [&](float (&fa)[8], float (&fb)[4], int buf, int sl) {
    const float* a_s = As + buf * (4 * QT) + sl * 128;
    const float* b_s = Ys + buf * QT + sl * 128 + b_off;
#pragma unroll
    for (int t = 0; t < 4; ++t) {
      fa[t] = a_s[a_off0 + t * T6_PLANE];
      fa[4 + t] = a_s[a_off1 + t * T6_PLANE];
      fb[t] = b_s[t * T6_PLANE];
    }
  };
  auto mfma8 = [&](const float (&fa)[8], const float (&fb)[4]) {
#pragma unroll
    for (int i = 0; i < 8; ++i) acc[i] = __builtin_amdgcn_mfma_f32_32x32x2f32(fa[i], fb[i & 3], acc[i], 0, 0, 0);
  };
#pragma unroll
  for (int i = 0; i < 8; ++i) fac[i] = 0.f;
#pragma unroll
  for (int i = 0; i < 4; ++i) fbc[i] = 0.f;
  const bool summer = p.colsum != nullptr && mi == 0 && wave == 0;
  float bsum = 0.f;
  issue(0);
  issue(1);
  issue(2);
  __builtin_amdgcn_s_waitcnt(0x0078);
  __builtin_amdgcn_s_barrier();
  asm volatile("" ::: "memory");
  for (int s = 0; s < nsteps; ++s) {
    const int buf = s & (NA - 1);
    __builtin_amdgcn_sched_barrier(0);
    issue(s + 3);
    load_frag(fa0, fb0, buf, 0);
    mfma8(fac, fbc);
    load_frag(fa1, fb1, buf, 1);
    mfma8(fa0, fb0);
    load_frag(fac, fbc, buf, 2);
    mfma8(fa1, fb1);
    __builtin_amdgcn_sched_group_barrier(0x100, 6, 0);
#pragma unroll
    for (int t = 0; t < 24; ++t) {
      __builtin_amdgcn_sched_group_barrier(0x008, 1, 0);
      if (t < 4) __builtin_amdgcn_sched_group_barrier(0x010, 1, 0);
      if (t >= 4 && t < 16) __builtin_amdgcn_sched_group_barrier(0x100, 1, 0);
    }
    __builtin_amdgcn_sched_barrier(0);
    if (summer) {
      const float* y1 = Ys + buf * QT + T6_PLANE;
#pragma unroll
      for (int hx = 0; hx < T6_H; ++hx) bsum += y1[hx * 64 + (lane ^ ((hx & 1) << 5))];
    }
    __builtin_amdgcn_s_waitcnt(0x0078);
    __builtin_amdgcn_s_barrier();
    asm volatile("" ::: "memory");
  }
  mfma8(fac, fbc);
  if (summer) p.colsum[(long long)z * p.Ndim + n0 + lane] = bsum;
  float* out = p.slab + (long long)z * p.slab_stride;
  const int col = n0 + wn * 32 + lr;
#pragma unroll
  for (int i = 0; i < 8; ++i)
#pragma unroll
    for (int e = 0; e < 16; ++e) {
      const int m = m0 + wm * 64 + (i >> 2) * 32 + (e & 3) + 8 * (e >> 2) + 4 * lh;
      out[((long long)(i0 + (i & 3)) * p.Mdim + m) * (long long)p.ldc + col] = acc[i][e];
    }
}

__global__ __launch_bounds__(256, 4) void wino63_unpool_yvd_kernel(const float* __restrict__ G, const uint32_t* __restrict__ bits,
                                                                 float* __restrict__ Y, float* __restrict__ Vd, long long nhex,
                                                                 long long g_rows, int hps, int g_tp, int Tvalid, int C, int ldg,
                                                                 int ld_bits, int ldv) {
  const int tpp = C >> 1;
  const long long idx = (long long)blockIdx.x * blockDim.x + threadIdx.x;
  const long long pair = idx / tpp;
  const int tl_ = (int)(idx - pair * tpp);
  const int half = tl_ & 1, hpar = (tl_ >> 1) & 1, kc = tl_ >> 2;
  const int c = 8 * kc + 4 * half;
  const long long hg = 2 * pair + hpar;
  if (hg >= nhex) return;
  const long long seq = hg / hps;
  const int hs = (int)(hg - seq * hps);
  const long long row0 = seq * g_tp + 3LL * hs;
// ... 257 lines not shown
  const long long n = ((nhex + 1) / 2) * (C / 2);
  TL_REQUIRE((n + 255) / 256 < (1LL << 31), "wino63_unpool_yvd: grid too large");
  hipLaunchKernelGGL(wino63_unpool_yvd_kernel, dim3((unsigned)((n + 255) / 256)), dim3(256), 0, (hipStream_t)stream, G, bits, Y, Vd,
                     nhex, (long long)g_rows, Tp / 6, g_tp, Tvalid, C, ldg, ld_bits, ldv);
  return check_launch("wino63_unpool_yvd");
}

extern "C" int tl_wino63_weights7(const float* w, float* fwd, int O, int I, int taps, void* stream) {
  using namespace tl;
  TL_REQUIRE(w && fwd && O > 0 && I > 0 && I % 8 == 0 && taps >= 7 && taps <= 9, "wino63_weights7: I %% 8 == 0 and 7..9 taps needed");
  const long long n = 3LL * O * I;
  TL_REQUIRE((n + 255) / 256 < (1LL << 31), "wino63_weights7: grid too large");
  hipLaunchKernelGGL(wino63_weights7_kernel, dim3((unsigned)((n + 255) / 256)), dim3(256), 0, (hipStream_t)stream, w, fwd, O, I, taps);
  return check_launch("wino63_weights7");
}

extern "C" int tl_wino63_xform2(const float* P, float* V0, float* V1, int64_t rows, int Tp, int Tvalid, int C, int ldp, int ldv,
                                void* stream) {
  using namespace tl;
  TL_REQUIRE(P && V0 && V1, "wino63_xform2: null pointer");
  TL_REQUIRE(Tp > 0 && Tp % 6 == 0 && rows > 0 && rows % Tp == 0 && Tvalid >= 0 && Tvalid <= Tp, "wino63_xform2: Tp %% 6 == 0, whole sequences, Tvalid <= Tp needed");
  TL_REQUIRE(C > 0 && C % 8 == 0 && ldp >= C && ldp % 4 == 0 && ldv >= C && ldv % 8 == 0, "wino63_xform2: C %% 8, ldp %% 4, ldv %% 8 needed");
  const long long nhex = rows / 6;
  const long long n = ((nhex + 1) / 2) * (C / 2);
  TL_REQUIRE((n + 255) / 256 < (1LL << 31), "wino63_xform2: grid too large");
  hipLaunchKernelGGL(wino63_xform2_kernel, dim3((unsigned)((n + 255) / 256)), dim3(256), 0, (hipStream_t)stream, P, V0, V1, nhex,
                     Tp / 6, Tp, Tvalid, C, ldp, ldv, 0);
  return check_launch("wino63_xform2");
}

extern "C" int tl_wino63_xform2s(const float* P, float* V0, float* V1, int64_t rows, int Tp, int Tvalid, int shift, int C, int ldp,
                                 int ldv, void* stream) {
  using namespace tl;
  TL_REQUIRE(P && V0 && V1, "wino63_xform2s: null pointer");
  TL_REQUIRE(Tp > 0 && Tp % 6 == 0 && rows > 0 && rows % Tp == 0 && Tvalid >= 0 && Tvalid <= Tp, "wino63_xform2s: Tp %% 6 == 0, whole sequences, Tvalid <= Tp needed");
  TL_REQUIRE(shift >= 0 && shift <= 6, "wino63_xform2s: shift must lie in 0..6");
  TL_REQUIRE(C > 0 && C % 8 == 0 && ldp >= C && ldp % 4 == 0 && ldv >= C && ldv % 8 == 0, "wino63_xform2s: C %% 8, ldp %% 4, ldv %% 8 needed");
  const long long nhex = rows / 6;
  const long long n = ((nhex + 1) / 2) * (C / 2);
  TL_REQUIRE((n + 255) / 256 < (1LL << 31), "wino63_xform2s: grid too large");
  hipLaunchKernelGGL(wino63_xform2_kernel, dim3((unsigned)((n + 255) / 256)), dim3(256), 0, (hipStream_t)stream, P, V0, V1, nhex,
                     Tp / 6, Tp, Tvalid, C, ldp, ldv, shift);
  return check_launch("wino63_xform2s");
}

extern "C" int tl_wino63_ydz(const float* G, float* Y, int64_t rows, int Tp, int Tvalid, int C, int ldg, int ldv, void* stream) {
  using namespace tl;
  TL_REQUIRE(G && Y, "wino63_ydz: null pointer");
  TL_REQUIRE(Tp > 0 && Tp % 6 == 0 && rows > 0 && rows % Tp == 0 && Tvalid >= 0 && Tvalid <= Tp, "wino63_ydz: Tp %% 6 == 0, whole sequences, Tvalid <= Tp needed");
  TL_REQUIRE(C > 0 && C % 8 == 0 && ldg >= C && ldg % 4 == 0 && ldv >= C && ldv % 8 == 0, "wino63_ydz: C %% 8, ldg %% 4, ldv %% 8 needed");
  const long long nhex = rows / 6;
  const long long n = ((nhex + 1) / 2) * (C / 2);
  TL_REQUIRE((n + 255) / 256 < (1LL << 31), "wino63_ydz: grid too large");
  hipLaunchKernelGGL(wino63_ydz_kernel, dim3((unsigned)((n + 255) / 256)), dim3(256), 0, (hipStream_t)stream, G, Y, nhex, Tp / 6, Tp,
                     Tvalid, C, ldg, ldv);
  return check_launch("wino63_ydz");
}

extern "C" int tl_conv7_wino63v_nt(const tl_nt_params* pp, void* stream) {
  using namespace tl;
  TL_REQUIRE(pp != nullptr, "conv7_wino63: null params");
  const tl_nt_params& p = *pp;
  TL_REQUIRE(p.A && p.aux && p.Bw && p.out, "conv7_wino63: null V0 (A) / V1 (aux) / Bw / out");
  TL_REQUIRE(p.loader == W_LOAD_V && p.epilogue == W_EPI_LRELU && p.row_shift == 0 && p.splitk <= 1,
             "conv7_wino63: loader 2 (pre-transformed operands), LRELU epilogue, row_shift 0, no split-K");
  TL_REQUIRE(p.J >= 7 && p.J <= 9, "conv7_wino63: 7..9 taps (three segments)");
  TL_REQUIRE(p.M > 0 && p.M % 6 == 0 && p.N > 0 && p.N % 32 == 0 && p.K >= 16 && p.K % 8 == 0, "conv7_wino63: M %% 6, N %% 32, K %% 8, K >= 16 needed");
  TL_REQUIRE(p.lda >= p.K && p.lda % 8 == 0 && p.ldb >= 3 * p.K && p.ldb % 8 == 0 && p.ldo >= p.N, "conv7_wino63: bad leading dimensions");
  TL_REQUIRE(p.A_rows % 2 == 0 && p.Tp > 0 && p.Tp % 6 == 0 && p.M % p.Tp == 0, "conv7_wino63: V holds hex pairs; Tp %% 6, whole sequences");
  TL_REQUIRE(8LL * p.N * p.ldb * 4 < (1LL << 31), "conv7_wino63: tap set larger than a buffer resource");
  TL_REQUIRE(128LL * 8 * p.lda * 4 + 4LL * p.K < (1LL << 31) && p.M + V6_ROWS < (1LL << 31), "conv7_wino63: tile span / M too large");
  TL_REQUIRE(p.slope >= 0.f && p.slope <= 1.f, "conv7_wino63: LeakyReLU slope must lie in [0, 1]");
  const long long ntm = (p.M + V6_ROWS - 1) / V6_ROWS;
  const long long nwg = ntm * ((p.N + V6_BN - 1) / V6_BN);
  TL_REQUIRE(nwg < (1LL << 31), "conv7_wino63: grid too large");
  TL_REQUIRE(p.A_rows >= ntm * V6_BH, "conv7_wino63: V0 / V1 must hold whole 128-hex tiles (pad them with zero hexes)");
  const long long ngrid = nwg < 256 ? nwg : 256;
  hipLaunchKernelGGL((wino63v_nt_kernel<W_EPI_LRELU>), dim3((unsigned)ngrid), dim3(512), 0, (hipStream_t)stream, p);
  return check_launch("conv7_wino63");
}

extern "C" int tl_conv7_wino63v_dgrad_nt(const tl_nt_params* pp, void* stream) {
  using namespace tl;
  TL_REQUIRE(pp != nullptr, "conv7_wino63_dgrad: null params");
  const tl_nt_params& p = *pp;
  TL_REQUIRE(p.A && p.aux && p.Bw && p.out, "conv7_wino63_dgrad: null V0 (A) / V1 (aux) / Bw / out");
  TL_REQUIRE(p.loader == W_LOAD_V && p.epilogue == W_EPI_MASK && p.row_shift == 0 && p.splitk <= 1,
             "conv7_wino63_dgrad: loader 2 (pre-transformed operands), MASK epilogue, row_shift 0 (the rows are moved by the transform), no split-K");
  TL_REQUIRE((p.auxbits != nullptr) != (p.mask != nullptr), "conv7_wino63_dgrad: exactly one mask source - auxbits (sign words) or mask (float rows)");
  TL_REQUIRE(p.J == 7, "conv7_wino63_dgrad: 7 taps");
  TL_REQUIRE(p.M > 0 && p.M % 6 == 0 && p.N > 0 && p.N % 32 == 0 && p.K >= 16 && p.K % 8 == 0, "conv7_wino63_dgrad: M %% 6, N %% 32, K %% 8, K >= 16 needed");
  TL_REQUIRE(p.lda >= p.K && p.lda % 8 == 0 && p.ldb >= 3 * p.K && p.ldb % 8 == 0 && p.ldo >= p.N, "conv7_wino63_dgrad: bad leading dimensions");
  TL_REQUIRE(p.auxbits == nullptr || p.ld_auxbits * 32 >= p.N, "conv7_wino63_dgrad: ld_auxbits too small");
  TL_REQUIRE(p.mask == nullptr || p.ld_mask >= p.N, "conv7_wino63_dgrad: ld_mask too small");
  TL_REQUIRE(p.A_rows % 2 == 0 && p.Tp > 0 && p.Tp % 6 == 0 && p.M % p.Tp == 0, "conv7_wino63_dgrad: V holds hex pairs; Tp %% 6, whole sequences");
  TL_REQUIRE(8LL * p.N * p.ldb * 4 < (1LL << 31), "conv7_wino63_dgrad: tap set larger than a buffer resource");
  TL_REQUIRE(128LL * 8 * p.lda * 4 + 4LL * p.K < (1LL << 31) && p.M + V6_ROWS < (1LL << 31), "conv7_wino63_dgrad: tile span / M too large");
  TL_REQUIRE(192LL * (p.ldo > p.ld_mask ? p.ldo : p.ld_mask) * 4 < (1LL << 31), "conv7_wino63_dgrad: ldo / ld_mask too large");
  TL_REQUIRE(p.slope >= 0.f && p.slope <= 1.f, "conv7_wino63_dgrad: LeakyReLU slope must lie in [0, 1]");
  const long long ntm = (p.M + V6_ROWS - 1) / V6_ROWS;
  const long long nwg = ntm * ((p.N + V6_BN - 1) / V6_BN);
  TL_REQUIRE(nwg < (1LL << 31), "conv7_wino63_dgrad: grid too large");
  TL_REQUIRE(p.A_rows >= ntm * V6_BH, "conv7_wino63_dgrad: V0 / V1 must hold whole 128-hex tiles (pad them with zero hexes)");
  const long long ngrid = nwg < 256 ? nwg : 256;
  if (p.auxbits != nullptr) hipLaunchKernelGGL((wino63v_nt_kernel<W6_EPI_MASK7>), dim3((unsigned)ngrid), dim3(512), 0, (hipStream_t)stream, p);
  else hipLaunchKernelGGL((wino63v_nt_kernel<W6_EPI_MASK7F>), dim3((unsigned)ngrid), dim3(512), 0, (hipStream_t)stream, p);
  return check_launch("conv7_wino63_dgrad");
}

extern "C" int tl_wino63_nt_tile_rows(void) { return tl::V6_ROWS; }

extern "C" int tl_conv3_wino63v_nt(const tl_nt_params* pp, void* stream) {
  using namespace tl;
  TL_REQUIRE(pp != nullptr, "wino63v_nt: null params");
  const tl_nt_params& p = *pp;
  TL_REQUIRE(p.A && p.Bw && (p.out || p.epilogue == W_EPI_C1W || p.epilogue == W_EPI_POOLV || p.epilogue == W_EPI_MASKY), "wino63v_nt: null V/Bw/out");
  TL_REQUIRE(p.loader == W_LOAD_V, "wino63v_nt: loader 2 (pre-transformed operand) only");
  TL_REQUIRE(p.J == 3 && p.splitk <= 1, "wino63v_nt: 3 taps, no split-K");
  TL_REQUIRE(p.M > 0 && p.M % 6 == 0 && p.N > 0 && p.K >= 40 && p.K % 8 == 0, "wino63v_nt: M %% 6, K %% 8, K >= 40 needed");
  TL_REQUIRE(p.lda >= p.K && p.ldb >= p.K && p.lda % 8 == 0 && p.ldb % 8 == 0, "wino63v_nt: bad leading dimensions (multiples of 8)");
  TL_REQUIRE(p.A_rows % 2 == 0, "wino63v_nt: V holds hex pairs");
  TL_REQUIRE(p.Tp > 0 && p.Tp % 6 == 0 && p.M % p.Tp == 0, "wino63v_nt: Tp must be a positive multiple of 6, M whole sequences");
  TL_REQUIRE(8LL * p.N * p.ldb * 4 < (1LL << 31), "wino63v_nt: tap set larger than a buffer resource");
  TL_REQUIRE(128LL * 8 * p.lda * 4 + 4LL * p.K < (1LL << 31), "wino63v_nt: tile span too large");
  const long long ntm = (p.M + V6_ROWS - 1) / V6_ROWS;
  const long long nwg = ntm * ((p.N + V6_BN - 1) / V6_BN);
  TL_REQUIRE(nwg < (1LL << 31), "wino63v_nt: grid too large");
  TL_REQUIRE(p.N % 32 == 0 && p.M + V6_ROWS < (1LL << 31), "wino63v_nt: N %% 32 == 0 and M < 2^31 - 768 needed");
  TL_REQUIRE(p.slope >= 0.f && p.slope <= 1.f, "wino63v_nt: LeakyReLU slope must lie in [0, 1]");
  TL_REQUIRE(p.A_rows >= ntm * V6_BH, "wino63v_nt: V must hold whole 128-hex tiles (pad it with zero hexes)");
  hipStream_t st = (hipStream_t)stream;
  const long long ngrid = nwg < 256 ? nwg : 256;
  if (p.epilogue == W_EPI_POOL) {
    TL_REQUIRE(p.row_shift == 0 && p.out && p.ldo >= p.N, "wino63v_nt: forward needs row_shift 0 and an output");
    TL_REQUIRE(p.obits != nullptr && p.Tvalid % 2 == 0 && p.Tvalid <= p.Tp, "wino63v_nt: POOL needs obits and an even Tvalid");
    TL_REQUIRE(p.ld_obits * 32 >= p.N, "wino63v_nt: POOL: ld_obits too small");
    TL_REQUIRE(p.out_tp >= 0 && (p.out_tp == 0 || 2 * p.out_tp >= p.Tvalid), "wino63v_nt: out_tp must cover the valid pooled rows");
    const long long orows = (p.M / p.Tp) * (long long)(p.out_tp > 0 ? p.out_tp : p.Tp / 2);
    TL_REQUIRE(orows * (long long)p.ldo * 4 < (1LL << 40), "wino63v_nt: output too large");
    hipLaunchKernelGGL((wino63v_nt_kernel<W_EPI_POOL>), dim3((unsigned)ngrid), dim3(512), 0, st, p);
  } else if (p.epilogue == W_EPI_POOLV) {
    TL_REQUIRE(p.row_shift == 0 && (p.out == nullptr || p.ldo >= p.N), "wino63v_nt: forward needs row_shift 0");
    TL_REQUIRE(p.obits != nullptr && p.Tvalid % 2 == 0 && p.Tvalid <= p.Tp, "wino63v_nt: POOLV needs obits and an even Tvalid");
    TL_REQUIRE(p.ld_obits * 32 >= p.N && p.Tp % 12 == 0, "wino63v_nt: POOLV needs Tp %% 12 == 0 (output hexes inside one sequence)");
    TL_REQUIRE(p.vout && p.vhalo && p.ld_vout >= p.N && p.ld_vout % 8 == 0 && p.vout_quads >= p.M / 12 && p.vout_quads % 2 == 0,
               "wino63v_nt: POOLV needs vout (>= M / 12 hexes, whole pairs, ld_vout %% 8 == 0) and vhalo");
    TL_REQUIRE(64LL * 8 * p.ld_vout * 4 < (1LL << 31), "wino63v_nt: ld_vout too large");
    hipLaunchKernelGGL((wino63v_nt_kernel<W_EPI_POOLV>), dim3((unsigned)ngrid), dim3(512), 0, st, p);
  } else if (p.epilogue == W_EPI_MASK) {
    TL_REQUIRE(p.row_shift == -2 && p.ldo >= p.N, "wino63v_nt: input gradient needs row_shift -2");
    TL_REQUIRE(p.auxbits != nullptr, "wino63v_nt: MASK needs auxbits (the sign bits of the stage input)");
    hipLaunchKernelGGL((wino63v_nt_kernel<W_EPI_MASK>), dim3((unsigned)ngrid), dim3(512), 0, st, p);
  } else if (p.epilogue == W_EPI_MASKY) {
    TL_REQUIRE(p.row_shift == -2 && p.auxbits != nullptr && p.abits != nullptr, "wino63v_nt: epilogue 6 needs row_shift -2, auxbits and abits");
    TL_REQUIRE(p.ld_abits * 32 >= p.N && p.Tvalid_in % 2 == 0 && p.Tvalid_in <= 2 * p.Tp, "wino63v_nt: epilogue 6: bad abits / Tvalid_in");
    TL_REQUIRE(p.vout && p.ld_vout >= p.N && p.ld_vout % 8 == 0 && p.vout_quads >= p.M / 3 && p.vout_quads % 2 == 0,
               "wino63v_nt: epilogue 6 needs vout (>= M / 3 hexes, whole pairs, ld_vout %% 8 == 0)");
    TL_REQUIRE((p.vout2 == nullptr) == (p.vhalo == nullptr), "wino63v_nt: epilogue 6 takes vout2 and vhalo together (Y and Vd) or neither (Y only)");
    TL_REQUIRE(128LL * 8 * p.ld_vout * 4 < (1LL << 31), "wino63v_nt: ld_vout too large");
    if (p.vout2 != nullptr) hipLaunchKernelGGL((wino63v_nt_kernel<W_EPI_MASKY>), dim3((unsigned)ngrid), dim3(512), 0, st, p);
    else hipLaunchKernelGGL((wino63v_nt_kernel<W6_EPI_MASKY_Y>), dim3((unsigned)ngrid), dim3(512), 0, st, p);
  } else if (p.epilogue == W_EPI_C1W) {
    TL_REQUIRE(p.row_shift == -2 || p.row_shift == 0, "wino63v_nt: epilogue 4 needs row_shift -2 (operand Vd) or 0 (operand Y)");
    TL_REQUIRE(p.auxbits && p.c1x && p.c1bits && p.c1partial, "wino63v_nt: epilogue 4 needs auxbits, c1x, c1bits, c1partial");
    TL_REQUIRE(p.c1kt >= 1 && p.c1kt <= 3 && p.c1T >= 2 * p.Tvalid + 2, "wino63v_nt: epilogue 4: 1..3 taps, c1T >= 2*Tvalid + 2");
    TL_REQUIRE(p.Tvalid >= 0 && p.Tvalid <= p.Tp, "wino63v_nt: epilogue 4: Tvalid must lie in [0, Tp]");
    if (p.row_shift == -2) hipLaunchKernelGGL((wino63v_nt_kernel<W_EPI_C1W>), dim3((unsigned)ngrid), dim3(512), 0, st, p);
    else hipLaunchKernelGGL((wino63v_nt_kernel<W6_EPI_C1W_Y>), dim3((unsigned)ngrid), dim3(512), 0, st, p);
  } else {
    set_error("wino63v_nt: unsupported epilogue %d", p.epilogue);
    return TL_EINVAL;
  }
  return check_launch("wino63v_nt");
}

extern "C" int tl_wino63_unpool_rows6(const float* G, const uint32_t* bits, float* A, int64_t rows, int64_t g_rows, int Tp, int g_tp,
                                      int Tvalid, int C, int ldg, int ld_bits, int lda, int pad, void* stream) {
  using namespace tl;
  TL_REQUIRE(G && bits && A, "wino63_unpool_rows6: null pointer");
  TL_REQUIRE(rows > 0 && Tp > 0 && rows % Tp == 0 && Tvalid > 0 && Tvalid <= Tp, "wino63_unpool_rows6: whole sequences of Tp rows, 0 < Tvalid <= Tp needed");
  TL_REQUIRE(g_tp > 0 && 2 * g_tp >= Tvalid && g_rows >= (rows / Tp) * (long long)g_tp, "wino63_unpool_rows6: G holds fewer rows than sequences x g_tp");
  TL_REQUIRE(C > 0 && C % 8 == 0 && ldg >= C && ldg % 4 == 0 && lda >= C && lda % 8 == 0 && ld_bits * 32 >= C,
             "wino63_unpool_rows6: C %% 8, ldg %% 4, lda %% 8 needed, bits row must cover C");
  const long long nhex = (rows + 5) / 6;
  const long long n = (nhex + 1) / 2 * (C >> 1);
  TL_REQUIRE((n + 255) / 256 < (1LL << 31), "wino63_unpool_rows6: grid too large");
  hipLaunchKernelGGL(wino63_unpool_rows6_kernel, dim3((unsigned)((n + 255) / 256)), dim3(256), 0, (hipStream_t)stream, G, bits, A,
                     nhex, (long long)rows, (long long)g_rows, Tp, g_tp, Tvalid, C, ldg, ld_bits, lda, pad);
  return check_launch("wino63_unpool_rows6");
}

extern "C" int tl_wino63_weights1(const float* w, float* taps, int O, int I, int ldb, void* stream) {
  using namespace tl;
  TL_REQUIRE(w && taps && O > 0 && I > 0 && ldb >= O && ldb % 8 == 0, "wino63_weights1: w, taps, O, I > 0 and ldb %% 8 == 0, ldb >= O needed");
  const long long n = (long long)ldb * 8 * I;
  TL_REQUIRE((n + 255) / 256 < (1LL << 31), "wino63_weights1: too large");
  hipLaunchKernelGGL(wino63_weights1_kernel, dim3((unsigned)((n + 255) / 256)), dim3(256), 0, (hipStream_t)stream, w, taps, O, I, ldb);
  return check_launch("wino63_weights1");
}

extern "C" int tl_conv1_wino63v_dgrad_nt(const tl_nt_params* pp, void* stream) {
  using namespace tl;
  TL_REQUIRE(pp != nullptr, "conv1_wino63v_dgrad_nt: null params");
  const tl_nt_params& p = *pp;
  TL_REQUIRE(p.A && p.Bw, "conv1_wino63v_dgrad_nt: null A / taps");
  TL_REQUIRE(p.loader == W_LOAD_V && p.epilogue == W_EPI_GY && p.J == 1 && p.row_shift == 0 && p.splitk <= 1,
             "conv1_wino63v_dgrad_nt: loader 2, epilogue 7, one tap, row_shift 0, no split-K");
  TL_REQUIRE(p.M > 0 && p.N > 0 && p.K >= 40 && p.K % 8 == 0, "conv1_wino63v_dgrad_nt: K %% 8, K >= 40 needed");
  TL_REQUIRE(p.Tp > 0 && p.Tp % 3 == 0 && p.M % p.Tp == 0, "conv1_wino63v_dgrad_nt: Tp (rows per sequence) must be a multiple of 3, M whole sequences");
  TL_REQUIRE(p.lda >= p.K && p.ldb >= p.K && p.lda % 8 == 0 && p.ldb % 8 == 0, "conv1_wino63v_dgrad_nt: bad leading dimensions (multiples of 8)");
  TL_REQUIRE(p.A_rows % 2 == 0, "conv1_wino63v_dgrad_nt: A holds hex pairs");
  TL_REQUIRE(8LL * p.N * p.ldb * 4 < (1LL << 31), "conv1_wino63v_dgrad_nt: tap set larger than a buffer resource");
  TL_REQUIRE(128LL * 8 * p.lda * 4 + 4LL * p.K < (1LL << 31), "conv1_wino63v_dgrad_nt: tile span too large");
  const long long ntm = (p.M + V6_ROWS - 1) / V6_ROWS;
  const long long nwg = ntm * ((p.N + V6_BN - 1) / V6_BN);
  TL_REQUIRE(nwg < (1LL << 31), "conv1_wino63v_dgrad_nt: grid too large");
  TL_REQUIRE(p.N % 32 == 0 && p.M + V6_ROWS < (1LL << 31), "conv1_wino63v_dgrad_nt: N %% 32 == 0 and M < 2^31 - 768 needed");
  TL_REQUIRE(p.slope >= 0.f && p.slope <= 1.f, "conv1_wino63v_dgrad_nt: LeakyReLU slope must lie in [0, 1]");
  TL_REQUIRE(p.A_rows >= ntm * V6_BH, "conv1_wino63v_dgrad_nt: A must hold whole 128-hex tiles (pad it with zero hexes)");
  TL_REQUIRE(p.auxbits != nullptr && p.abits != nullptr, "conv1_wino63v_dgrad_nt: needs auxbits (sign) and abits (arg-max) of the stage below");
  TL_REQUIRE(p.out_tp > 0 && p.out_tp <= p.Tp && 2 * p.out_tp >= p.Tvalid_in, "conv1_wino63v_dgrad_nt: out_tp = rows per sequence of the bit arrays (0 < out_tp <= Tp, covering Tvalid_in / 2)");
  TL_REQUIRE(p.ld_abits * 32 >= p.N && p.ld_auxbits * 32 >= p.N && p.Tvalid_in % 2 == 0 && p.Tvalid_in <= 2 * p.Tp, "conv1_wino63v_dgrad_nt: bad abits / auxbits / Tvalid_in");
  TL_REQUIRE(p.vout && p.vout2 && p.vhalo && p.ld_vout >= p.N && p.ld_vout % 8 == 0 && p.vout_quads >= p.M / 3 && p.vout_quads % 2 == 0,
             "conv1_wino63v_dgrad_nt: needs vout / vout2 (>= M / 3 hexes, whole pairs, ld_vout %% 8 == 0) and vhalo");
  TL_REQUIRE(128LL * 8 * p.ld_vout * 4 < (1LL << 31), "conv1_wino63v_dgrad_nt: ld_vout too large");
  const long long ngrid = nwg < 256 ? nwg : 256;
  hipLaunchKernelGGL((wino63v_nt_kernel<W_EPI_GY>), dim3((unsigned)ngrid), dim3(512), 0, (hipStream_t)stream, p);
  return check_launch("conv1_wino63v_dgrad_nt");
}

extern "C" int tl_conv3_wino63v_tn(const tl_tn_params* pp, void* stream) {
  using namespace tl;
  TL_REQUIRE(pp != nullptr, "wino63v_tn: null params");
  tl_tn_params p = *pp;
  if (p.splitk < 1) p.splitk = 1;
  if (p.loader == 3) {
    TL_REQUIRE(p.A && p.B && p.slab, "wino63v_tn: null V/Y/slab");
    TL_REQUIRE(p.J == 3 && p.Tp > 0 && p.Tp % 6 == 0 && p.Krows > 0 && p.Krows % p.Tp == 0, "wino63v_tn: loader 3: bad Tp / Krows");
    TL_REQUIRE(p.Krows + 64 < (1LL << 31), "wino63v_tn: more than 2^31 reduction rows");
    TL_REQUIRE(p.Mdim % 256 == 0 && p.Ndim % 64 == 0 && p.lda % 8 == 0 && p.ldb % 8 == 0 && p.lda >= p.Mdim && p.ldb >= p.Ndim &&
               p.ldc >= p.Ndim, "wino63v_tn: loader 3 needs Mdim %% 256, Ndim %% 64, lda / ldb %% 8");
    TL_REQUIRE(p.A_rows % 2 == 0 && p.B_rows % 2 == 0 && p.vd == nullptr, "wino63v_tn: loader 3: whole hex pairs in V and Y, no Vd");
    TL_REQUIRE(p.a_hex == 0 || p.a_hex == 1, "wino63v_tn: loader 3: a_hex must be 0 or 1");
    TL_REQUIRE(p.splitk <= 65535 && (p.splitk == 1 || p.slab_stride >= 8LL * p.Mdim * p.ldc), "wino63v_tn: bad splitk / slab_stride");
    const long long ks = (p.Krows / 6 + T6_H - 1) / T6_H;
    TL_REQUIRE(p.A_rows >= ks * T6_H && p.B_rows >= ks * T6_H, "wino63v_tn: V and Y must hold whole 6-hex K-steps (pad with zero hexes)");
    const long long per3 = (ks + p.splitk - 1) / p.splitk;
    TL_REQUIRE((per3 + 4) * (long long)T6_H * 8 * p.lda * 4 < (1LL << 31) && (per3 + 4) * (long long)T6_H * 8 * p.ldb * 4 < (1LL << 31),
               "wino63v_tn: a reduction split spans more than 2 GB of V or Y: raise splitk");
    const int ntm3 = p.Mdim / 256;
    hipLaunchKernelGGL(wino63v_tn4y_kernel, dim3((unsigned)(2 * ntm3 * (p.Ndim / T6_BN)), (unsigned)p.splitk, 1), dim3(512), 0,
                       (hipStream_t)stream, p, ntm3);
    return check_launch("wino63v_tn (both operands pre-transformed)");
  }
  TL_REQUIRE(p.A && p.B && p.slab && p.bbits, "wino63v_tn: null V/B/bbits/slab");
  TL_REQUIRE(p.a_hex == 0, "wino63v_tn: a_hex needs loader 3 (both operands pre-transformed)");
  TL_REQUIRE(p.J == 3 && p.loader == 1, "wino63v_tn: 3 taps, UNPOOL loader (1) or pre-transformed Y (3)");
  TL_REQUIRE(p.Tp > 0 && p.Tp % 6 == 0 && p.Tvalid % 2 == 0 && p.Tvalid <= p.Tp, "wino63v_tn: Tp %% 6 == 0 and an even Tvalid <= Tp needed");
  TL_REQUIRE(p.Krows > 0 && p.Krows % p.Tp == 0 && p.Mdim > 0 && p.Ndim > 0, "wino63v_tn: bad sizes (Krows must be whole sequences)");
  TL_REQUIRE(p.Krows + 64 < (1LL << 31), "wino63v_tn: more than 2^31 reduction rows");
  TL_REQUIRE(p.Mdim % 128 == 0 && p.Ndim % 64 == 0 && p.lda % 8 == 0 && p.ldb % 4 == 0 && p.A_rows % 2 == 0,
             "wino63v_tn: Mdim %% 128, Ndim %% 64, lda %% 8, ldb %% 4, whole hex pairs in V needed");
  TL_REQUIRE(p.lda >= p.Mdim && p.ldb >= p.Ndim && p.ldc >= p.Ndim, "wino63v_tn: leading dimension too small");
  TL_REQUIRE(p.ld_bbits * 32 >= p.Ndim && p.ld_bbits % 2 == 0, "wino63v_tn: bbits row too short / odd");
  TL_REQUIRE(p.splitk <= 65535, "wino63v_tn: splitk too large");
  TL_REQUIRE(p.splitk == 1 || p.slab_stride >= 8LL * p.Mdim * p.ldc, "wino63v_tn: slab_stride smaller than 8*Mdim*ldc");
  const int g_tp = p.g_tp > 0 ? p.g_tp : p.Tp / 2;
  TL_REQUIRE(2 * g_tp >= p.Tvalid, "wino63v_tn: g_tp must cover the valid pooled rows");
  TL_REQUIRE(p.B_rows >= (p.Krows / p.Tp) * (long long)g_tp && p.B_rows < (1LL << 30), "wino63v_tn: G holds fewer rows than sequences x g_tp");
  const long long ksteps_all = (p.Krows / 6 + T6_H - 1) / T6_H;
  TL_REQUIRE(p.A_rows >= (ksteps_all + 3) * T6_H, "wino63v_tn: V must hold whole 6-hex K-steps and three more (pad it with zero hexes)");
  const long long per = (ksteps_all + p.splitk - 1) / p.splitk;
  TL_REQUIRE((per + 4) * (long long)T6_H * 8 * p.lda * 4 < (1LL << 31), "wino63v_tn: a reduction split spans more than 2 GB of V: raise splitk");
  TL_REQUIRE((per + 6) * 3LL * T6_H * p.ldb * 4 < (1LL << 31), "wino63v_tn: a reduction split spans more than 2 GB of G: raise splitk");
  TL_REQUIRE(p.vd == nullptr || (p.ld_vd >= p.Ndim && p.ld_vd % 8 == 0), "wino63v_tn: ld_vd must cover Ndim (multiple of 8)");
  TL_REQUIRE(p.vd == nullptr || (per + 4) * (long long)T6_H * 8 * p.ld_vd * 4 < (1LL << 31), "wino63v_tn: a reduction split spans more than 2 GB of Vd: raise splitk");
  const int ntn = p.Ndim / T6_BN;
  hipStream_t st = (hipStream_t)stream;
  TL_REQUIRE(p.bm == 0 || p.bm == 128 || (p.bm == 256 && p.Mdim % 256 == 0 && p.Tp >= 12),
             "wino63v_tn: bm must be 0, 128, or 256 with Mdim %% 256 == 0 and Tp >= 12");
  if (p.bm == 256 || (p.bm == 0 && p.Mdim % 256 == 0 && p.Tp >= 12)) {
    const int ntm = p.Mdim / 256;
    const dim3 grid((unsigned)(2 * ntm * ntn), (unsigned)p.splitk, 1);
    if (p.vd != nullptr) hipLaunchKernelGGL((wino63v_tn4_kernel<true>), grid, dim3(512), 0, st, p, ntm);
    else hipLaunchKernelGGL((wino63v_tn4_kernel<false>), grid, dim3(512), 0, st, p, ntm);
    return check_launch("wino63v_tn (4 transforms per workgroup)");
  }
  const int ntm = p.Mdim / 128;
  const dim3 grid((unsigned)(ntm * ntn), (unsigned)p.splitk, 1);
  if (p.vd != nullptr) hipLaunchKernelGGL((wino63v_tn_kernel<true>), grid, dim3(512), 0, st, p, ntm);
  else hipLaunchKernelGGL((wino63v_tn_kernel<false>), grid, dim3(512), 0, st, p, ntm);
  return check_launch("wino63v_tn");
}

extern "C" int tl_conv1_fwd_v6(const float* x, const float* w, const float* b, float* P, float* V, uint32_t* bits, uint32_t* sign,
                               int64_t S, int T, int ktaps, int C1, int Tp, int Tout, float slope, void* stream) {
  using namespace tl;
  TL_REQUIRE(x && w && b && V && bits, "conv1_fwd_v6: null pointer");
  TL_REQUIRE(S > 0 && S < (1LL << 31) && T > 0, "conv1_fwd_v6: bad sizes");
  TL_REQUIRE(ktaps >= 1 && ktaps <= C1_MAXKT, "conv1_fwd_v6: ktaps must be 1..%d", C1_MAXKT);
  TL_REQUIRE(C1 % 128 == 0 && C1 <= 1024 && (C1 & (C1 - 1)) == 0, "conv1_fwd_v6: C1 must be 128, 256, 512 or 1024");
  TL_REQUIRE(Tp > 0 && Tp % 6 == 0, "conv1_fwd_v6: Tp must be a multiple of 6");
  TL_REQUIRE(Tout >= 0 && Tout <= Tp && 2 * Tout + ktaps - 1 <= T, "conv1_fwd_v6: Tout/Tp/T inconsistent (%d,%d,%d)", Tout, Tp, T);
  TL_REQUIRE((size_t)T * 4 <= 64 * 1024, "conv1_fwd_v6: T too large for the LDS window");
#define TL_C1V_LAUNCH(KT_)                                                                                                   \
  case KT_:                                                                                                                  \
    hipLaunchKernelGGL(conv1_fwd_vh_kernel<KT_>, dim3((unsigned)S), dim3(256), (size_t)T * 4, (hipStream_t)stream, x, w, b, P, V, \
                       bits, sign, (long long)S, T, C1, Tp, Tout, slope);                                                    \
    break;
  switch (ktaps) {
    TL_C1V_LAUNCH(1) TL_C1V_LAUNCH(2) TL_C1V_LAUNCH(3) TL_C1V_LAUNCH(4) TL_C1V_LAUNCH(5) TL_C1V_LAUNCH(6) TL_C1V_LAUNCH(7)
    TL_C1V_LAUNCH(8)
  }
#undef TL_C1V_LAUNCH
  return check_launch("conv1_fwd_v6");
}
```

### decode_tonal_langauge_amd/csrc/tonal_wino63_epi.h

```cpp
#pragma once
#include "tonal_common.h"
#include "tonal_wino43_epi.h"
#include "tonal_wino43v_epi.h"

namespace tl {

enum { W6_EPI_MASKY_Y = 8, W6_EPI_C1W_Y = 9, W6_EPI_MASK7 = 10, W6_EPI_MASK7F = 11 };

constexpr unsigned V6_DROP = 0x80000000u;
constexpr unsigned long long V6_HI = 0xffffffff00000000ull;

template <bool IMM>
__device__ __forceinline__ void v6_store_at(float x, __amdgpu_buffer_rsrc_t rs, unsigned vo, unsigned so, unsigned k) {
  if constexpr (IMM) __builtin_amdgcn_raw_buffer_store_b32(__builtin_bit_cast(unsigned, x), rs, vo + k, so, 0);
  else __builtin_amdgcn_raw_buffer_store_b32(__builtin_bit_cast(unsigned, x), rs, vo, so + k, 0);
}

__device__ __forceinline__ void v6_pair_swap(float& a, float& b) {
  const auto r = __builtin_amdgcn_permlane32_swap(__float_as_uint(a), __float_as_uint(b), false, false);
  a = __uint_as_float(r[0]);
  b = __uint_as_float(r[1]);
}

template <bool IMM>
__device__ __forceinline__ void v6_store_hex_pair(float (&ha)[8], float (&hb)[8], __amdgpu_buffer_rsrc_t rs, unsigned voAP, unsigned voAQ,
                                                  unsigned voBP, unsigned voBQ, unsigned so) {
#pragma unroll
  for (int i = 0; i < 8; ++i) v6_pair_swap(ha[i], hb[i]);
#pragma unroll
  for (int t = 0; t < 8; t += 2) {
    {
      const auto r = __builtin_amdgcn_permlane16_swap(__float_as_uint(ha[t]), __float_as_uint(ha[t + 1]), false, false);
      v6_store_at<IMM>(__uint_as_float(r[0]), rs, voAP, so, (unsigned)(t * 64));
      v6_store_at<IMM>(__uint_as_float(r[1]), rs, voAQ, so, (unsigned)(t * 64));
    }
    {
      const auto r = __builtin_amdgcn_permlane16_swap(__float_as_uint(hb[t]), __float_as_uint(hb[t + 1]), false, false);
      v6_store_at<IMM>(__uint_as_float(r[0]), rs, voBP, so, (unsigned)(t * 64));
      v6_store_at<IMM>(__uint_as_float(r[1]), rs, voBQ, so, (unsigned)(t * 64));
    }
  }
}
__device__ __forceinline__ unsigned v6_pair_offset(int colbase, int lr, int lh) {
  return (unsigned)((colbase >> 3) + ((lr >> 3) & 1)) * 512u + (unsigned)((lr >> 4) & 1) * 64u + (unsigned)lh * 32u + (unsigned)(lr & 7) * 4u;
}

__device__ __forceinline__ void wino63_rows(const f32x16 (&acc)[8], int e, float (&y)[6]) {
  const float m1 = acc[1][e], m2 = acc[2][e], m3 = acc[3][e], m4 = acc[4][e], m5 = acc[5][e], m6 = acc[6][e];
  const float a12 = m1 + m2, s12 = m1 - m2, a34 = m3 + m4, s34 = m3 - m4, a56 = m5 + m6, s56 = m5 - m6;
  y[0] = ((acc[0][e] + a12) + a34) + a56;
  y[1] = fmaf(0.5f, s56, fmaf(2.f, s34, s12));
  y[2] = fmaf(0.25f, a56, fmaf(4.f, a34, a12));
  y[3] = fmaf(0.125f, s56, fmaf(8.f, s34, s12));
  y[4] = fmaf(0.0625f, a56, fmaf(16.f, a34, a12));
  y[5] = fmaf(0.03125f, s56, fmaf(32.f, s34, s12)) + acc[7][e];
}
__device__ __forceinline__ void wino63_bt(const float (&d)[8], float (&v)[8]) {
  v[0] = fmaf(5.25f, d[2] - d[4], d[6] - d[0]);
  const float e1 = fmaf(-4.25f, d[4], d[2] + d[6]), o1 = fmaf(-4.25f, d[3], d[1] + d[5]);
  v[1] = e1 + o1;
  v[2] = e1 - o1;
  const float e2 = fmaf(0.25f, d[2], fmaf(-1.25f, d[4], d[6])), o2 = fmaf(0.5f, d[1], fmaf(-2.5f, d[3], 2.f * d[5]));
  v[3] = e2 + o2;
  v[4] = e2 - o2;
  const float e3 = fmaf(4.f, d[2], fmaf(-5.f, d[4], d[6])), o3 = fmaf(2.f, d[1], fmaf(-2.5f, d[3], 0.5f * d[5]));
  v[5] = e3 + o3;
  v[6] = e3 - o3;
  v[7] = fmaf(5.25f, d[3] - d[5], d[7] - d[1]);
}
__device__ __forceinline__ void wino63_b(const float (&m)[8], float (&d)[8]) {
  const float a12 = m[1] + m[2], s12 = m[1] - m[2], a34 = m[3] + m[4], s34 = m[3] - m[4], a56 = m[5] + m[6], s56 = m[5] - m[6];
  d[0] = -m[0];
  d[1] = fmaf(2.f, s56, fmaf(0.5f, s34, s12)) - m[7];
  d[2] = fmaf(5.25f, m[0], fmaf(4.f, a56, fmaf(0.25f, a34, a12)));
  d[3] = fmaf(5.25f, m[7], fmaf(-2.5f, s34 + s56, -4.25f * s12));
  d[4] = fmaf(-5.25f, m[0], fmaf(-5.f, a56, fmaf(-1.25f, a34, -4.25f * a12)));
  d[5] = fmaf(-5.25f, m[7], fmaf(0.5f, s56, fmaf(2.f, s34, s12)));
  d[6] = ((m[0] + a12) + a34) + a56;
  d[7] = m[7];
}

__device__ __forceinline__ float selbit(uint32_t w, int j, float a, float b) {
  const uint32_t m = (uint32_t)__builtin_amdgcn_sbfe((int)w, j, 1);
  return __uint_as_float((__float_as_uint(a) & m) | (__float_as_uint(b) & ~m));
}

struct v6_rows {
  int tA, tB;
  long long seqA, seqB;
};
__device__ __forceinline__ v6_rows v6_rows_of(long long Hw, int Tp) {
  v6_rows r;
  const unsigned R = (unsigned)(6 * Hw);
  const unsigned s = R / (unsigned)Tp;
  r.seqA = (long long)(unsigned)__builtin_amdgcn_readfirstlane((int)s);
  r.tA = __builtin_amdgcn_readfirstlane((int)(R - s * (unsigned)Tp));
  r.tB = r.tA + 96;
  r.seqB = r.seqA;
  while (r.tB >= Tp) {
    r.tB -= Tp;
    ++r.seqB;
  }
  return r;
}
struct bits96 {
  unsigned long long lo;
  uint32_t hi;
};
__device__ __forceinline__ unsigned long long mask96(const bits96& a, const bits96& b, int j) {
  return j < 64 ? mask2l(a.lo, b.lo, j) : mask2(a.hi, b.hi, j - 64);
}
__device__ __forceinline__ bits96 v6_in_bits96(long long R0h, long long M) {
  bits96 r;
  r.lo = v5_in_bits<64, 1>(R0h, M);
  r.hi = (uint32_t)v5_in_bits<32, 1>(R0h + 64, M);
  return r;
}
__device__ __forceinline__ bits96 v6_valid_bits96(int t0, int Tp, int tlim, long long R0h, long long M) {
  bits96 r;
  r.lo = v5_valid_bits<64, 1>(t0, Tp, tlim, R0h, M);
  int t1 = t0 + 64;
  while (t1 >= Tp) t1 -= Tp;
  r.hi = (uint32_t)v5_valid_bits<32, 1>(t1, Tp, tlim, R0h + 64, M);
  return r;
}

template <bool VOUT, bool FULL>
__device__ __forceinline__ void v6_epilogue_pool(const tl_nt_params& p, const f32x16 (&acc)[8], const v5_pre_pool& pre, float* xch,
                                                 long long R0, int n0, int wm, int wn, int lr_in, int lh, long long tm) {
  int lr = lr_in;
  asm volatile("" : "+v"(lr));
  const int colbase = n0 + wn * 32;
  const bool colok = colbase < p.N;
  const int col = colbase + lr;
  const long long Hw = tm * 128 + wm * 32;
  const int Tp = p.Tp, Tq = Tp >> 1;
  const v6_rows rw = v6_rows_of(Hw, Tp);
  const unsigned long long vA = v5_valid_bits<48, 2>(rw.tA, Tp, p.Tvalid, 6 * Hw, p.M);
  const unsigned long long vB = v5_valid_bits<48, 2>(rw.tB, Tp, p.Tvalid, 6 * Hw + 96, p.M);
  const float bv = pre.bv;
  const long long P0 = 3 * Hw;
  const long long prows = p.M >> 1;
  const int out_tp = (!VOUT && p.out_tp > 0) ? p.out_tp : Tq;
  const int tqa0 = rw.tA >> 1, tqb0 = rw.tB >> 1;
  const unsigned long long kA = v5_valid_bits<48, 1>(tqa0, Tq, out_tp, P0, prows);
  const unsigned long long kB = v5_valid_bits<48, 1>(tqb0, Tq, out_tp, P0 + 48, prows);
  const long long nseq = p.M / Tp;
  const long long obase = rw.seqA * out_tp;
  const __amdgpu_buffer_rsrc_t rsO = rsrc_of(!VOUT ? p.out + obase * (long long)p.ldo : nullptr,
                                            !VOUT ? (nseq * out_tp - obase) * (long long)p.ldo * 4 : 0);
  const unsigned ldo4 = (unsigned)p.ldo * 4u;
  const unsigned col4 = colok ? (unsigned)col * 4u : V6_DROP;
  int ta = tqa0, tb = tqb0;
  unsigned ra = (unsigned)tqa0 * ldo4, rb = ((unsigned)(rw.seqB - rw.seqA) * (unsigned)out_tp + (unsigned)tqb0) * ldo4;
  const unsigned seq_step = (unsigned)(out_tp - Tq) * ldo4;
  float pv[48];
  uint32_t wb0 = 0, wb1 = 0, ws0 = 0, ws1 = 0;
  static_for<0, 16>([&](auto E) {
    constexpr int e = decltype(E)::value;
    float y[6];
    wino63_rows(acc, e, y);
    unsigned vo_e = 0;
    if constexpr (!VOUT) vo_e = selmu(V6_HI, rb, ra) + col4;
    static_for<0, 3>([&](auto H) {
      constexpr int h = decltype(H)::value, j = 3 * e + h;
      const float y0 = lrelu01(y[2 * h] + bv, p.slope), y1 = lrelu01(y[2 * h + 1] + bv, p.slope);
      const bool valid = __builtin_amdgcn_inverse_ballot_w64(mask2l(vA, vB, j));
      const bool gt = (y1 > y0) && valid;
      const float o = valid ? (gt ? y1 : y0) : 0.f;
      pv[j] = o;
      if constexpr (j < 32) {
        wb0 = wb0 + wb0 + (uint32_t)gt;
        ws0 = ws0 + ws0 + (uint32_t)(o > 0.f);
      } else {
        wb1 = wb1 + wb1 + (uint32_t)gt;
        ws1 = ws1 + ws1 + (uint32_t)(o > 0.f);
      }
      if constexpr (!VOUT) {
        const unsigned vo = selmu(mask2l(kA, kB, j), vo_e, V5_OOB);
        __builtin_amdgcn_raw_buffer_store_b32(__builtin_bit_cast(unsigned, o), rsO, vo, (unsigned)h * ldo4, 0);
      }
    });
    if constexpr (!VOUT) {
      ta += 3;
      ra += 3u * ldo4;
      const bool wa = ta >= Tq;
      ta -= wa ? Tq : 0;
      ra += wa ? seq_step : 0u;
      tb += 3;
      rb += 3u * ldo4;
      const bool wbb = tb >= Tq;
      tb -= wbb ? Tq : 0;
      rb += wbb ? seq_step : 0u;
    }
  });
  {
    wb0 = bit_transpose32(__builtin_bitreverse32(wb0), lr);
    ws0 = bit_transpose32(__builtin_bitreverse32(ws0), lr);
    wb1 = bit_transpose32(__builtin_bitreverse32(wb1) >> 16, lr);
    ws1 = bit_transpose32(__builtin_bitreverse32(ws1) >> 16, lr);
    const long long wleft = (nseq * out_tp - obase) * (long long)p.ld_obits * 4;
    const long long wbase = obase * (long long)p.ld_obits + (colbase >> 5);
    const __amdgpu_buffer_rsrc_t rsB = rsrc_of(p.obits + wbase, wleft - (long long)(colbase >> 5) * 4);
    const __amdgpu_buffer_rsrc_t rsS = rsrc_of(p.osign ? p.osign + wbase : nullptr, p.osign ? wleft - (long long)(colbase >> 5) * 4 : 0);
    const unsigned t0h = (unsigned)(lh ? tqb0 : tqa0);
    const unsigned s0h = lh ? (unsigned)(rw.seqB - rw.seqA) : 0u;
#pragma unroll
    for (int b = 0; b < 2; ++b) {
      const unsigned r = 32u * b + (unsigned)lr;
      unsigned t = t0h + r;
      const unsigned c = t / (unsigned)Tq;
      t -= c * (unsigned)Tq;
      const bool keep = colok && r < 48u && t < (unsigned)out_tp && (P0 + 48 * lh + r) < prows;
      const unsigned wo = keep ? ((s0h + c) * (unsigned)out_tp + t) * (unsigned)p.ld_obits * 4u : V5_OOB;
      __builtin_amdgcn_raw_buffer_store_b32(b ? wb1 : wb0, rsB, wo, 0u, 0);
      __builtin_amdgcn_raw_buffer_store_b32(b ? ws1 : ws0, rsS, wo, 0u, 0);
    }
  }
  if constexpr (VOUT) {
    if (p.out != nullptr) {
      const __amdgpu_buffer_rsrc_t rsP = rsrc_of(p.out + P0 * (long long)p.ldo, (prows - P0) * (long long)p.ldo * 4);
      const unsigned pvoff = colok ? ((unsigned)(48 * lh) * (unsigned)p.ldo + (unsigned)col) * 4u : V5_OOB;
#pragma unroll
      for (int j = 0; j < 48; ++j) {
        const unsigned vo = selmu(mask2l(kA, kB, j), pvoff, V5_OOB);
        __builtin_amdgcn_raw_buffer_store_b32(__builtin_bit_cast(unsigned, pv[j]), rsP, vo, (unsigned)j * (unsigned)p.ldo * 4u, 0);
      }
    }
    const int slot = wm * 2 + lh;
    {
      float2 v2 = {pv[0], pv[1]};
      *reinterpret_cast<float2*>(xch + (slot * 64 + wn * 32 + lr) * 2) = v2;
    }
    __builtin_amdgcn_s_waitcnt(0xc07f);
    __builtin_amdgcn_s_barrier();
    asm volatile("" ::: "memory");
    float nb0 = 0.f, nb1 = 0.f;
    if (slot < 7) {
      const float2 v2 = *reinterpret_cast<const float2*>(xch + ((slot + 1) * 64 + wn * 32 + lr) * 2);
      nb0 = v2.x;
      nb1 = v2.y;
    }
    uint32_t seA = 0, seB = 0, nvA = 0, nvB = 0;
    {
      int t_a = tqa0, t_b = tqb0;
      const long long qa = (Hw >> 1), qb = (Hw >> 1) + 8;
      for (int k = 0; k < 8; ++k) {
        seA |= (uint32_t)(t_a == Tq - 6) << k;
        seB |= (uint32_t)(t_b == Tq - 6) << k;
        nvA |= (uint32_t)(FULL || qa + k < p.vout_quads) << k;
        nvB |= (uint32_t)(FULL || qb + k < p.vout_quads) << k;
        t_a += 6;
        if (t_a >= Tq) t_a -= Tq;
        t_b += 6;
        if (t_b >= Tq) t_b -= Tq;
      }
    }
    const long long Hn = Hw >> 1;
    const __amdgpu_buffer_rsrc_t rsV = rsrc_of(p.vout + Hn * 8 * (long long)p.ld_vout,
                                              (p.vout_quads - Hn) * 8 * (long long)p.ld_vout * 4);
    const unsigned pair4 = (unsigned)p.ld_vout * 64u;
    const unsigned offP = v6_pair_offset(colbase, lr, lh);
    const unsigned vvA = colok ? offP : V6_DROP, vvB = colok ? 4u * pair4 + offP : V6_DROP;
    const unsigned long long mraw = wm == 3 ? V6_HI : 0ull;
#pragma unroll
    for (int qp = 0; qp < 4; ++qp) {
      float vv[2][8];
#pragma unroll
      for (int hq = 0; hq < 2; ++hq) {
        const int q = 2 * qp + hq;
        const unsigned long long mend = mask2(seA, seB, q);
        float d[8];
#pragma unroll
        for (int k = 0; k < 6; ++k) d[k] = pv[6 * q + k];
        d[6] = selm(mend, 0.f, q < 7 ? pv[(6 * q + 6) % 48] : nb0);
        d[7] = selm(mend, 0.f, q < 7 ? pv[(6 * q + 7) % 48] : nb1);
        wino63_bt(d, vv[hq]);
        if (q == 7) {
#pragma unroll
          for (int k = 0; k < 6; ++k) vv[hq][k] = selm(mraw, d[k], vv[hq][k]);
        }
      }
      const int q = 2 * qp;
      const unsigned voA = selmu(mask2(nvA, nvA >> 1, q), vvA, V6_DROP), voB = selmu(mask2(nvB, nvB >> 1, q), vvB, V6_DROP);
      v6_store_hex_pair<FULL>(vv[0], vv[1], rsV, voA, voA + 1024u, voB, voB + 1024u, (unsigned)qp * pair4);
    }
    {
      const bool hw = wm == 0 && p.vhalo != nullptr;
      const __amdgpu_buffer_rsrc_t rsH = rsrc_of(hw ? p.vhalo + tm * 2 * (long long)p.N : nullptr, hw ? 2LL * p.N * 4 : 0);
      const unsigned ho = (colok && lh == 0) ? (unsigned)col * 4u : V5_OOB;
      __builtin_amdgcn_raw_buffer_store_b32(__builtin_bit_cast(unsigned, pv[0]), rsH, ho, 0u, 0);
      __builtin_amdgcn_raw_buffer_store_b32(__builtin_bit_cast(unsigned, pv[1]), rsH, ho, (unsigned)p.N * 4u, 0);
    }
  }
}

template <int EPI>
constexpr int v6_stores() {
  return EPI == W_EPI_POOL ? 52 : EPI == W_EPI_POOLV ? 70
         : (EPI == W_EPI_MASK || EPI == W_EPI_LRELU || EPI == W6_EPI_MASK7 || EPI == W6_EPI_MASK7F) ? 96
         : (EPI == W_EPI_MASKY || EPI == W6_EPI_MASKY_Y || EPI == W_EPI_GY) ? 63 : 0;
}

struct v6_pre_mask {
  uint32_t s[3];
};
__device__ __forceinline__ v6_pre_mask v6_prefetch_mask(const tl_nt_params& p, long long R0, int n0, int wm, int wn, int lr, int lh) {
  const int colbase = n0 + wn * 32;
  const long long ra = R0 + wm * 192 + 96 * lh + lr;
  v6_pre_mask r = {{0u, 0u, 0u}};
#pragma unroll
  for (int k = 0; k < 3; ++k)
    if (colbase < p.N && ra + 32 * k < p.M) r.s[k] = p.auxbits[(ra + 32 * k) * (long long)p.ld_auxbits + (colbase >> 5)];
  return r;
}
template <bool FULL, bool FMASK = false>
__device__ __forceinline__ void v6_epilogue_mask(const tl_nt_params& p, const f32x16 (&acc)[8], const v6_pre_mask& pre, long long R0,
                                                 int n0, int wm, int wn, int lr_in, int lh) {
  int lr = lr_in;
  asm volatile("" : "+v"(lr));
  const int colbase = n0 + wn * 32;
  const bool colok = colbase < p.N;
  const int col = colbase + lr;
  const long long Rw = R0 + wm * 192;
  const __amdgpu_buffer_rsrc_t rsO = rsrc_of(p.out + Rw * (long long)p.ldo, (p.M - Rw) * (long long)p.ldo * 4);
  const unsigned ovoff = colok ? ((unsigned)(96 * lh) * (unsigned)p.ldo + (unsigned)col) * 4u : V5_OOB;
  const unsigned ldo4 = (unsigned)p.ldo * 4u;
  bits96 inA = {~0ull, ~0u}, inB = inA;
  if (!FULL) {
    inA = v6_in_bits96(Rw, p.M);
    inB = v6_in_bits96(Rw + 96, p.M);
  }
  uint32_t sT[3] = {0u, 0u, 0u};
  if constexpr (!FMASK) {
#pragma unroll
    for (int k = 0; k < 3; ++k) sT[k] = bit_transpose32(pre.s[k], lr);
  }
  const __amdgpu_buffer_rsrc_t rsM = rsrc_of(FMASK ? p.mask + Rw * (long long)p.ld_mask : p.out, FMASK ? (p.M - Rw) * (long long)p.ld_mask * 4 : 0);
  const unsigned mvoff = (FMASK && colok) ? ((unsigned)(96 * lh) * (unsigned)p.ld_mask + (unsigned)col) * 4u : V5_OOB;
  const unsigned ldm4 = (unsigned)p.ld_mask * 4u;
#pragma unroll
  for (int e = 0; e < 16; ++e) {
    float y[6];
    wino63_rows(acc, e, y);
#pragma unroll
    for (int h = 0; h < 6; ++h) {
      const int r = 6 * e + h;
      float o;
      if constexpr (FMASK) {
        const unsigned mo = FULL ? mvoff : selmu(mask96(inA, inB, r), mvoff, V5_OOB);
        const float x = __builtin_bit_cast(float, __builtin_amdgcn_raw_buffer_load_b32(rsM, mo, (unsigned)r * ldm4, 0));
        o = y[h] * (x > 0.f ? 1.f : p.slope);
      } else {
        o = y[h] * selbit(sT[r >> 5], r & 31, 1.f, p.slope);
      }
      const unsigned vo = FULL ? ovoff : selmu(mask96(inA, inB, r), ovoff, V5_OOB);
      __builtin_amdgcn_raw_buffer_store_b32(__builtin_bit_cast(unsigned, o), rsO, vo, (unsigned)r * ldo4, 0);
    }
  }
}

template <bool FULL>
__device__ __forceinline__ void v6_epilogue_lrelu(const tl_nt_params& p, const f32x16 (&acc)[8], const v5_pre_pool& pre, long long R0,
                                                  int n0, int wm, int wn, int lr_in, int lh) {
  int lr = lr_in;
  asm volatile("" : "+v"(lr));
  const int colbase = n0 + wn * 32;
  const bool colok = colbase < p.N;
  const int col = colbase + lr;
  const long long Rw = R0 + wm * 192;
  const __amdgpu_buffer_rsrc_t rsO = rsrc_of(p.out + Rw * (long long)p.ldo, (p.M - Rw) * (long long)p.ldo * 4);
  const unsigned ovoff = colok ? ((unsigned)(96 * lh) * (unsigned)p.ldo + (unsigned)col) * 4u : V5_OOB;
  const unsigned ldo4 = (unsigned)p.ldo * 4u;
  bits96 inA = {~0ull, ~0u}, inB = inA;
  if (!FULL) {
    inA = v6_in_bits96(Rw, p.M);
    inB = v6_in_bits96(Rw + 96, p.M);
  }
  const float bv = pre.bv;
#pragma unroll
  for (int e = 0; e < 16; ++e) {
    float y[6];
    wino63_rows(acc, e, y);
#pragma unroll
    for (int h = 0; h < 6; ++h) {
      const int r = 6 * e + h;
      const float o = lrelu01(y[h] + bv, p.slope);
      const unsigned vo = FULL ? ovoff : selmu(mask96(inA, inB, r), ovoff, V5_OOB);
      __builtin_amdgcn_raw_buffer_store_b32(__builtin_bit_cast(unsigned, o), rsO, vo, (unsigned)r * ldo4, 0);
    }
  }
}

struct v6_pre_masky {
  uint32_t s[3], a[3];
};
template <bool GTP = false>
__device__ __forceinline__ v6_pre_masky v6_prefetch_masky(const tl_nt_params& p, long long R0, int n0, int wm, int wn, int lr, int lh) {
  const int colbase = n0 + wn * 32;
  const long long ra = R0 + wm * 192 + 96 * lh + lr;
  v6_pre_masky r;
#pragma unroll
  for (int k = 0; k < 3; ++k) {
    r.s[k] = r.a[k] = 0u;
    if (colbase < p.N && ra + 32 * k < p.M) {
      long long row = ra + 32 * k;
      bool have = true;
      if constexpr (GTP) {
        const unsigned R = (unsigned)row, sq = R / (unsigned)p.Tp, t = R - sq * (unsigned)p.Tp;
        have = t < (unsigned)p.out_tp;
        row = (long long)sq * p.out_tp + t;
      }
      if (have) {
        r.s[k] = p.auxbits[row * (long long)p.ld_auxbits + (colbase >> 5)];
        r.a[k] = p.abits[row * (long long)p.ld_abits + (colbase >> 5)];
      }
    }
  }
  return r;
}
template <bool FULL, bool DIRECT = false, bool VD = true>
__device__ __forceinline__ void v6_epilogue_masky(const tl_nt_params& p, const f32x16 (&acc)[8], const v6_pre_masky& pre, float* xch,
                                                  long long R0, int n0, int wm, int wn, int lr_in, int lh, long long tm) {
  int lr = lr_in;
  asm volatile("" : "+v"(lr));
  const int colbase = n0 + wn * 32;
  const bool colok = colbase < p.N;
  const int col = colbase + lr;
  const long long Rw = R0 + wm * 192;
  const int Tp = p.Tp, hps = Tp / 3;
  const v6_rows rw = v6_rows_of(tm * 128 + wm * 32, Tp);
  uint32_t we[3], wo[3], sT[3], firstw = 0;
  (void)hps;
  {
    const bits96 okA = v6_valid_bits96(rw.tA, Tp, p.Tvalid_in >> 1, Rw, p.M);
    const bits96 okB = v6_valid_bits96(rw.tB, Tp, p.Tvalid_in >> 1, Rw + 96, p.M);
    const uint32_t okw[3] = {lh ? (uint32_t)okB.lo : (uint32_t)okA.lo, lh ? (uint32_t)(okB.lo >> 32) : (uint32_t)(okA.lo >> 32),
                             lh ? okB.hi : okA.hi};
    if constexpr (VD) {
      uint32_t fA = 0, fB = 0;
      int ha = rw.tA / 3, hb = rw.tB / 3;
      for (int k = 0; k < 32; ++k) {
        fA |= (uint32_t)(ha == 0) << k;
        fB |= (uint32_t)(hb == 0) << k;
        ha = ha + 1 == hps ? 0 : ha + 1;
        hb = hb + 1 == hps ? 0 : hb + 1;
      }
      firstw = lh ? fB : fA;
    }
#pragma unroll
    for (int k = 0; k < 3; ++k) {
      sT[k] = bit_transpose32(pre.s[k], lr);
      const uint32_t aT = bit_transpose32(pre.a[k], lr);
      we[k] = okw[k] & ~aT;
      wo[k] = okw[k] & aT;
    }
  }
  const long long Hb = Rw / 3;
  const unsigned pair4 = (unsigned)p.ld_vout * 64u;
  const __amdgpu_buffer_rsrc_t rsY = rsrc_of(p.vout + Hb * 8 * (long long)p.ld_vout, (p.vout_quads - Hb) * 8 * (long long)p.ld_vout * 4);
  const __amdgpu_buffer_rsrc_t rsD = rsrc_of(VD ? p.vout2 + Hb * 8 * (long long)p.ld_vout : nullptr,
                                            VD ? (p.vout_quads - Hb) * 8 * (long long)p.ld_vout * 4 : 0);
  const unsigned offP = v6_pair_offset(colbase, lr, lh);
  const unsigned vvA = colok ? offP : V6_DROP, vvB = colok ? 16u * pair4 + offP : V6_DROP;
  const int nexA = (int)(p.M / 3 - Hb < 64 ? p.M / 3 - Hb : 64) - lh, nexB = nexA - 32;
  float pe = 0.f, po = 0.f;
  float first_d[6], v1keep[8];
#pragma unroll
  for (int k = 0; k < 6; ++k) first_d[k] = 0.f;
#pragma unroll
  for (int k = 0; k < 8; ++k) v1keep[k] = 0.f;
  auto andf = [](float x, uint32_t m) { return __uint_as_float(__float_as_uint(x) & m); };
#pragma unroll
  for (int e = 0; e < 16; ++e) {
    float y[6];
    if constexpr (DIRECT) {
#pragma unroll
      for (int h = 0; h < 6; ++h) y[h] = acc[h][e];
    } else {
      wino63_rows(acc, e, y);
    }
    float dzr[12];
#pragma unroll
    for (int h = 0; h < 6; ++h) {
      const int r = 6 * e + h;
      const float t = y[h] * selbit(sT[r >> 5], r & 31, 1.f, p.slope);
      dzr[2 * h] = andf(t, (uint32_t)__builtin_amdgcn_sbfe((int)we[r >> 5], r & 31, 1));
      dzr[2 * h + 1] = andf(t, (uint32_t)__builtin_amdgcn_sbfe((int)wo[r >> 5], r & 31, 1));
    }
    float Yp[2][8], Vp[2][8];
#pragma unroll
    for (int hh = 0; hh < 2; ++hh) {
      const int j = 2 * e + hh;
      const float* d6 = dzr + 6 * hh;
      const float ev1 = (d6[0] + d6[2]) + d6[4], od1 = (d6[1] + d6[3]) + d6[5];
      const float ev2 = fmaf(16.f, d6[4], fmaf(4.f, d6[2], d6[0])), od2 = fmaf(32.f, d6[5], fmaf(8.f, d6[3], 2.f * d6[1]));
      const float ev3 = fmaf(0.0625f, d6[4], fmaf(0.25f, d6[2], d6[0])), od3 = fmaf(0.03125f, d6[5], fmaf(0.125f, d6[3], 0.5f * d6[1]));
      Yp[hh][0] = d6[0];
      Yp[hh][1] = ev1 + od1;
      Yp[hh][2] = ev1 - od1;
      Yp[hh][3] = ev2 + od2;
      Yp[hh][4] = ev2 - od2;
      Yp[hh][5] = ev3 + od3;
      Yp[hh][6] = ev3 - od3;
      Yp[hh][7] = d6[5];
      if constexpr (!VD) {
      } else if (j == 0) {
#pragma unroll
        for (int k = 0; k < 6; ++k) first_d[k] = d6[k];
      } else {
        const uint32_t keep = ~(uint32_t)__builtin_amdgcn_sbfe((int)firstw, j, 1);
        float d[8];
        d[0] = andf(pe, keep);
        d[1] = andf(po, keep);
#pragma unroll
        for (int k = 0; k < 6; ++k) d[2 + k] = d6[k];
        wino63_bt(d, Vp[hh]);
      }
      pe = d6[4];
      po = d6[5];
    }
    {
      const int j = 2 * e;
      const unsigned so = (unsigned)e * pair4;
      const unsigned voA = FULL ? vvA : (j < nexA ? vvA : V6_DROP), voB = FULL ? vvB : (j < nexB ? vvB : V6_DROP);
      v6_store_hex_pair<FULL>(Yp[0], Yp[1], rsY, voA, voA + 1024u, voB, voB + 1024u, so);
      if constexpr (!VD) {
      } else if (e == 0) {
#pragma unroll
        for (int i = 0; i < 8; ++i) v1keep[i] = Vp[1][i];
      } else {
        v6_store_hex_pair<FULL>(Vp[0], Vp[1], rsD, voA, voA + 1024u, voB, voB + 1024u, so);
      }
    }
    __builtin_amdgcn_sched_barrier(0);
  }
  if constexpr (VD) {
  const int slot = wm * 2 + lh;
  {
    float2 v2 = {pe, po};
    *reinterpret_cast<float2*>(xch + (slot * 64 + wn * 32 + lr) * 2) = v2;
  }
  __builtin_amdgcn_s_waitcnt(0xc07f);
  __builtin_amdgcn_s_barrier();
  asm volatile("" ::: "memory");
  {
    float fe = 0.f, fo = 0.f;
    if (slot > 0) {
      const float2 v2 = *reinterpret_cast<const float2*>(xch + ((slot - 1) * 64 + wn * 32 + lr) * 2);
      fe = v2.x;
      fo = v2.y;
    }
    const uint32_t keep = ~(uint32_t)__builtin_amdgcn_sbfe((int)firstw, 0, 1);
    float d[8], v[8];
    d[0] = andf(fe, keep);
    d[1] = andf(fo, keep);
#pragma unroll
    for (int k = 0; k < 6; ++k) d[2 + k] = first_d[k];
    wino63_bt(d, v);
    const bool raw = slot == 0;
#pragma unroll
    for (int k = 0; k < 8; ++k) v[k] = raw ? (k < 2 ? 0.f : d[k]) : v[k];
    const unsigned voA = FULL ? vvA : (0 < nexA ? vvA : V6_DROP), voB = FULL ? vvB : (0 < nexB ? vvB : V6_DROP);
    v6_store_hex_pair<FULL>(v, v1keep, rsD, voA, voA + 1024u, voB, voB + 1024u, 0u);
  }
  {
    const bool hw = wm == 3 && p.vhalo != nullptr;
    const __amdgpu_buffer_rsrc_t rsH = rsrc_of(hw ? p.vhalo + tm * 2 * (long long)p.N : nullptr, hw ? 2LL * p.N * 4 : 0);
    const unsigned ho = (colok && lh == 1) ? (unsigned)col * 4u : V5_OOB;
    __builtin_amdgcn_raw_buffer_store_b32(__builtin_bit_cast(unsigned, pe), rsH, ho, 0u, 0);
    __builtin_amdgcn_raw_buffer_store_b32(__builtin_bit_cast(unsigned, po), rsH, ho, (unsigned)p.N * 4u, 0);
  }
  }
}

struct v6_pre_c1w {
  uint32_t s[3], c[3];
  f32x4 x[2];
};
__device__ __forceinline__ v6_pre_c1w v6_prefetch_c1w(const tl_nt_params& p, long long R0, int n0, int wm, int wn, int lr, int lh) {
  const int colbase = n0 + wn * 32;
  const long long rh = R0 + wm * 192 + 96 * lh;
  v6_pre_c1w r;
  const int Tp = p.Tp;
  const long long nseq = p.M / Tp;
  const unsigned s0 = (unsigned)(R0 / Tp);
  const __amdgpu_buffer_rsrc_t rsX = rsrc_of(p.c1x + (long long)s0 * p.c1T, (nseq - s0) * (long long)p.c1T * 4);
  typedef unsigned v4u __attribute__((ext_vector_type(4)));
#pragma unroll
  for (int k = 0; k < 3; ++k) {
    r.s[k] = r.c[k] = 0u;
    const long long rk = rh + lr + 32 * k;
    if (colbase < p.N && rk < p.M) {
      r.s[k] = p.auxbits[rk * (long long)p.ld_auxbits + (colbase >> 5)];
      r.c[k] = p.c1bits[rk * (long long)p.ld_auxbits + (colbase >> 5)];
    }
  }
  const unsigned Rx = (unsigned)(rh + 3 * lr), sx = Rx / (unsigned)Tp, tx = Rx - sx * (unsigned)Tp;
  const unsigned xo = ((sx - s0) * (unsigned)p.c1T + 2u * tx) * 4u;
  r.x[0] = __builtin_bit_cast(f32x4, (v4u)__builtin_amdgcn_raw_buffer_load_b128(rsX, xo, 0u, 0));
  r.x[1] = __builtin_bit_cast(f32x4, (v4u)__builtin_amdgcn_raw_buffer_load_b128(rsX, xo + 16u, 0u, 0));
  return r;
}
template <bool YFORM = false>
__device__ __forceinline__ void v6_epilogue_c1w(const tl_nt_params& p, const f32x16 (&acc)[8], const v6_pre_c1w& pre, float* xw,
                                                float* red, long long R0, int n0, int wm, int wn, int lr_in, int lh, long long tm) {
  int lr = lr_in;
  asm volatile("" : "+v"(lr));
  const int colbase = n0 + wn * 32;
  const bool colok = colbase < p.N;
  const int col = colbase + lr;
  const long long Hw = tm * 128 + wm * 32;
  const long long Rw = 6 * Hw;
  const int Tp = p.Tp;
  const v6_rows rw = v6_rows_of(Hw, Tp);
  const bits96 okA = v6_valid_bits96(rw.tA, Tp, p.Tvalid, Rw, p.M);
  const bits96 okB = v6_valid_bits96(rw.tB, Tp, p.Tvalid, Rw + 96, p.M);
  float* xh = xw + lh * 256;
  *reinterpret_cast<f32x4*>(xh + 8 * lr) = pre.x[0];
  *reinterpret_cast<f32x4*>(xh + 8 * lr + 4) = pre.x[1];
  uint32_t keepw = ~0u;
  uint32_t okx0 = 0, okx1 = 0, sx0 = 0, sx1 = 0, cx0 = 0, cx1 = 0;
  f32x4 xx = {0.f, 0.f, 0.f, 0.f};
  float2 xy = {0.f, 0.f};
  if constexpr (YFORM) {
    const int hps = Tp / 6;
    auto starts = [hps](int t0) {
      uint32_t w = 0;
      for (int e = t0 == 0 ? 0 : hps - t0 / 6; e < 17; e += hps) w |= 1u << e;
// ... 92 lines not shown
```

Measured before the change: 1283 mel-frames/s.

## Run conv3 F(6,3) input gradient on Y3 and skip writing Vd3

Under the default nt63 mode, conv4's input-gradient kernel now writes only Y3, with no Vd3 and no Vd fixup pass. Conv3's input gradient then consumes Y3 directly through a new Y-operand MASKY epilogue, which applies the Winograd output transform in-kernel and carries overlap terms across tiles via LDS exchange, a halo buffer and a small fixup kernel. This removes the Vd3 buffer write/read and a fixup launch, at the cost of a heavier epilogue with an extra barrier and a new fixup kernel. The old behaviour is kept under an nt63vd option.

```diff
diff --git a/decode_tonal_langauge_amd/_conv_stack.py b/decode_tonal_langauge_amd/_conv_stack.py
--- a/decode_tonal_langauge_amd/_conv_stack.py
+++ b/decode_tonal_langauge_amd/_conv_stack.py
@@ -18,6 +18,20 @@
         self.tc = tin - k + 1
         self.tout = self.tc // 2 if pool else self.tc
         self.tp_out = tp_in // 2 if pool else tp_in
+
+
+class _HexStore(dict):
+
+    def __init__(self, stack):
+        super().__init__()
+        self._stack = stack
+
+    def __missing__(self, idx):
+        stack = self._stack
+        for st in stack.stages:
+            if st.idx == idx and stack._f63(st):
+                return stack._v_hex_buffer(self, idx, stack.S * st.tp_in, st.cout)
+        raise KeyError(idx)
 
 
 class ConvStack(LaunchTimers):
@@ -67,6 +81,7 @@
         self.wino43 = mode != "0"
         self.store_p1 = _kernels.get("store_p1") == "1"
         self.fuse_c1 = True
+        self.dgrad3_on_y = _kernels.get("conv4_dgrad") != "nt63vd"
         self.wino_vout = True
         self.tn_bm = 0
         self._gy_A = None
@@ -86,7 +101,7 @@
         self.Yt = {}
         self._y_ready = {}
         self.V = {}
-        self.Vd = {}
+        self.Vd = _HexStore(self)
         self._vd_ready = {}
         self.G = None
         return True
@@ -293,7 +308,7 @@
         if not (self.wino63 and self.f63_yprod3 and len(self.stages) >= 3):
             return False
         below, st = self.stages[1], self.stages[2]
-        return (_kernels.get("conv4_dgrad") == "nt63" and st.k == 1 and st.pool and self._f63(below)
+        return (_kernels.get("conv4_dgrad") in ("nt63", "nt63vd") and st.k == 1 and st.pool and self._f63(below)
                 and st.cout % 32 == 0 and st.cout >= 40 and st.cin % 32 == 0 and (below.tp_in // 2) % 3 == 0)
 
     def _stage_dgrad_gy(self, st, w):
@@ -316,31 +331,36 @@
         check(self.lib.tl_wino63_weights1(ptr(w), ptr(taps), st.cout, st.cin, st.cout, self._stream()), "tl_wino63_weights1")
         rows3 = S * below.tp_in
         Y3 = self._v_hex_buffer(self.Yt, below.idx, rows3, below.cout)
-        Vd3 = self._v_hex_buffer(self.Vd, below.idx, rows3, below.cout)
+        want_vd = not self._dgrad3_on_y() or self.store_p1
+        Vd3 = self._v_hex_buffer(self.Vd, below.idx, rows3, below.cout) if want_vd else None
         ntm = -(-rows // self._nt63_rows())
-        halo = self._halo_buffer("d3", ntm, below.cout)
+        halo = self._halo_buffer("d3", ntm, below.cout) if want_vd else None
         self._nt(tag=None, fn="tl_conv1_wino63v_dgrad_nt", A=ptr(A), A_rows=A.shape[0], lda=A.shape[2], loader=LOAD_V,
                  Bw=ptr(taps), M=rows, N=st.cin, K=st.cout, ldb=st.cout, ldo=st.cin, J=1, row_shift=0, Tp=tpg, slope=self.slope,
                  auxbits=ptr(self.sbits[below.idx]), ld_auxbits=self.sbits[below.idx].shape[1], abits=ptr(self.bits[below.idx]),
                  ld_abits=below.cout // 32, out_tp=below.tp_out, Tvalid_in=2 * below.tout, epilogue=EPI_GY, out=None,
                  vout=ptr(Y3), vout2=ptr(Vd3), vhalo=ptr(halo), vout_quads=Y3.shape[0], ld_vout=Y3.shape[2])
-        check(self.lib.tl_wino63_vd_fixup(ptr(Vd3), ptr(halo), rows // 3, ntm, below.tp_in // 6, below.cout, Vd3.shape[2],
-                                          self._stream()), "tl_wino63_vd_fixup")
+        if Vd3 is not None:
+            check(self.lib.tl_wino63_vd_fixup(ptr(Vd3), ptr(halo), rows // 3, ntm, below.tp_in // 6, below.cout, Vd3.shape[2],
+                                              self._stream()), "tl_wino63_vd_fixup")
         if ev:
             ev[1].record()
         self._y_ready[below.idx] = self.generation
         self._vd_ready[below.idx] = self.generation
         return None
 
+    def _dgrad3_on_y(self) -> bool:
+        return self.dgrad3_on_y and self.gy4 and self.f63_yprod
+
     def _stage_dgrad63(self, st, w):
         S = self.S
         rows_in = S * st.tp_in
         if self._vd_ready.get(st.idx) != self.generation:
-            raise RuntimeError("F(6,3) input gradient: its operand (Vd from the stage's weight-gradient pass, or Y2 from the "
-                               "input gradient of stage 3) must be written first")
+            raise RuntimeError("F(6,3) input gradient: its operand (Vd from the stage's weight-gradient pass, or Y from the "
+                               "input gradient of the stage above) must be written first")
         self._vd_ready[st.idx] = -1
-        on_y = st.idx == 2 and self.f63_yprod
-        Vd = self.Yt[2] if on_y else self.Vd[st.idx]
+        on_y = (st.idx == 2 and self.f63_yprod) or (st.idx == 3 and self._dgrad3_on_y())
+        Vd = self.Yt[st.idx] if on_y else self.Vd[st.idx]
         if on_y:
             wd = torch.empty(8, st.cin, st.cout, dtype=torch.float32, device=w.device)
             check(self.lib.tl_wino63_weights_y(ptr(w), ptr(wd), st.cout, st.cin, st.cout, self._stream()), "tl_wino63_weights_y")
@@ -356,9 +376,19 @@
             Vd2 = self._v_hex_buffer(self.Vd, 2, rows2, below.cout) if self.store_p1 else None
             ntm = -(-rows_in // self._nt63_rows())
             halo = self._halo_buffer("d2", ntm, below.cout) if self.store_p1 else None
-            self._nt(tag="conv3_dgrad", fn="tl_conv3_wino63v_nt", epilogue=EPI_MASKY, out=None, vout=ptr(Y2), vout2=ptr(Vd2),
-                     vhalo=ptr(halo), vout_quads=Y2.shape[0], ld_vout=Y2.shape[2], abits=ptr(self.bits[2]),
-                     ld_abits=below.cout // 32, Tvalid_in=2 * below.tout, **kw)
+            ykw = dict(epilogue=EPI_MASKY, out=None, vout_quads=Y2.shape[0], ld_vout=Y2.shape[2], abits=ptr(self.bits[2]),
+                       ld_abits=below.cout // 32, Tvalid_in=2 * below.tout)
+            if on_y:
+                self._nt(tag="conv3_dgrad", fn="tl_conv3_wino63v_nt", vout=ptr(Y2), vout2=None,
+                         vhalo=ptr(self._halo_buffer("y2", ntm, below.cout)), **ykw, **kw)
+                if Vd2 is not None:
+                    Vd3 = self.Vd[3]
+                    wv = self._pack_wino63(w, False)
+                    kw.update(A=ptr(Vd3), A_rows=Vd3.shape[0], lda=Vd3.shape[2], Bw=ptr(wv), row_shift=-2)
+                    Y2 = torch.zeros_like(Y2)
+            if not on_y or Vd2 is not None:
+                self._nt(tag=None if on_y else "conv3_dgrad", fn="tl_conv3_wino63v_nt", vout=ptr(Y2), vout2=ptr(Vd2),
+                         vhalo=ptr(halo), **ykw, **kw)
             if Vd2 is not None:
                 check(self.lib.tl_wino63_vd_fixup(ptr(Vd2), ptr(halo), rows_in // 3, ntm, below.tp_in // 6, below.cout,
                                                   Vd2.shape[2], self._stream()), "tl_wino63_vd_fixup")
@@ -441,13 +471,15 @@
             if self.f63_yprod3:
                 gy = self.gy4
                 src = "the epilogue of conv4's input gradient" if gy else "wino63_unpool_yvd_kernel"
-                fams[f"wino63v_tn4y_kernel (conv3 weight gradient, {f6}: both operands by LDS-DMA, no transform in the kernel; Y3 / Vd3 "
+                ops = "Y3" if self._dgrad3_on_y() and not self.store_p1 else "Y3 / Vd3"
+                fams[f"wino63v_tn4y_kernel (conv3 weight gradient, {f6}: both operands by LDS-DMA, no transform in the kernel; {ops} "
                      f"from {src})"] = ["conv3_wgrad"]
             else:
                 fams[f"{tn} (conv3 weight gradient, {f6}; also writes Vd)"] = ["conv3_wgrad"]
             if self.f63_yprod:
                 both = "Y and Vd" if self.store_p1 else "Y"
-                fams[f"wino63v_nt_kernel<MASKY> (conv3 input gradient, {f6}; writes {both} of conv2 instead of the gradient rows)"] = ["conv3_dgrad"]
+                on = "on Y3, " if self._dgrad3_on_y() else ""
+                fams[f"wino63v_nt_kernel<MASKY> (conv3 input gradient, {on}{f6}; writes {both} of conv2 instead of the gradient rows)"] = ["conv3_dgrad"]
                 fams[f"wino63v_tn4y_kernel (conv2 weight gradient, {f6}: both operands by LDS-DMA, no transform in the kernel)"] = ["conv2_wgrad"]
             else:
                 fams[f"wino63v_nt_kernel<MASK> (conv3 input gradient, {f6})"] = ["conv3_dgrad"]
diff --git a/decode_tonal_langauge_amd/_kernels.py b/decode_tonal_langauge_amd/_kernels.py
--- a/decode_tonal_langauge_amd/_kernels.py
+++ b/decode_tonal_langauge_amd/_kernels.py
@@ -23,9 +23,10 @@
     "f63_yprod": ("TONAL_F63_YPROD", _B, "1", "F(6,3): the backward operands of stages 2 and 3 (Y2 for both passes of stage 2; Y3 / Vd3) come "
                                               "pre-transformed out of the input-gradient epilogue of the stage above (0: the weight-gradient "
                                               "kernels un-pool and transform the gradient rows themselves and write Vd)"),
-    "conv4_dgrad": ("TONAL_CONV4_DGRAD", frozenset({"nt63", "gemm"}), "nt63",
-                    "F(6,3): the one-tap stage behind conv3 - nt63: its input gradient on the NT63 kernel, writing Y3 / Vd3 "
-                    "(no gradient rows, no tl_wino63_unpool_yvd); gemm: one-tap GEMM + tl_wino63_unpool_yvd"),
+    "conv4_dgrad": ("TONAL_CONV4_DGRAD", frozenset({"nt63", "nt63vd", "gemm"}), "nt63",
+                    "F(6,3): the one-tap stage behind conv3 - nt63: its input gradient on the NT63 kernel, writing Y3 (no gradient "
+                    "rows, no tl_wino63_unpool_yvd), and conv3's input gradient on that Y3; nt63vd: the same kernel writing Y3 and "
+                    "Vd3, conv3's input gradient on Vd3 (the A/B partner); gemm: one-tap GEMM + tl_wino63_unpool_yvd (Y3 and Vd3)"),
     "store_p1": ("TONAL_STORE_P1", _B, "0", "keep the raw pooled rows of stages 1 / 2 beside V, and Vd2 beside Y2 (tests)"),
     "conv7": ("TONAL_CONV7", frozenset({"wino63", "wino63bwd", "direct"}), "wino63",
               "the CNN-RNN classifier's 7-tap convolutions: wino63 three F(6,3) segments forward, direct kernels backward; "
diff --git a/decode_tonal_langauge_amd/csrc/tonal_wino63.hip b/decode_tonal_langauge_amd/csrc/tonal_wino63.hip
--- a/decode_tonal_langauge_amd/csrc/tonal_wino63.hip
+++ b/decode_tonal_langauge_amd/csrc/tonal_wino63.hip
@@ -224,7 +224,7 @@
 
 template <int EPI>
 __global__ __launch_bounds__(512, 2) void wino63v_nt_kernel(const tl_nt_params p) {
-  __shared__ __attribute__((aligned(1024))) char lds[3 * V6_STAGE + ((EPI == W_EPI_POOLV || EPI == W_EPI_MASKY || EPI == W_EPI_GY) ? 4096 : (EPI == W_EPI_C1W || EPI == W6_EPI_C1W_Y) ? 16384 : 0)];
+  __shared__ __attribute__((aligned(1024))) char lds[3 * V6_STAGE + ((EPI == W_EPI_POOLV || EPI == W_EPI_MASKY || EPI == W_EPI_GY || EPI == W6_EPI_MASKY_YY) ? 4096 : (EPI == W_EPI_C1W || EPI == W6_EPI_C1W_Y) ? 16384 : 0)];
   const int tid = threadIdx.x;
   const int lane = tid & 63;
   const int wave = __builtin_amdgcn_readfirstlane(tid >> 6);
@@ -235,7 +235,7 @@
   const long long ntm = (p.M + V6_ROWS - 1) / V6_ROWS;
   const long long nwg = ntm * ntn;
   constexpr bool SEG3 = EPI == W_EPI_LRELU || EPI == W6_EPI_MASK7 || EPI == W6_EPI_MASK7F;
-  constexpr bool SIX = EPI == W_EPI_GY;
+  constexpr bool SIX = EPI == W_EPI_GY || EPI == W6_EPI_GY_Y;
   const int kseg = p.K / V6_BK;
   const int nsteps = SEG3 ? 3 * kseg : kseg;
   f32x16 acc[8];
@@ -371,8 +371,8 @@
       if constexpr (EPI == W_EPI_POOL || EPI == W_EPI_POOLV || EPI == W_EPI_LRELU) return v5_prefetch_pool(p, cur.n0, wn, lr);
       else if constexpr (EPI == W_EPI_MASK || EPI == W6_EPI_MASK7) return v6_prefetch_mask(p, cur.R0, cur.n0, wm, wn, lr, lh);
       else if constexpr (EPI == W6_EPI_MASK7F) return v6_pre_mask{{0u, 0u, 0u}};
-      else if constexpr (EPI == W_EPI_MASKY || EPI == W6_EPI_MASKY_Y) return v6_prefetch_masky(p, cur.R0, cur.n0, wm, wn, lr, lh);
-      else if constexpr (EPI == W_EPI_GY) return v6_prefetch_masky<true>(p, cur.R0, cur.n0, wm, wn, lr, lh);
+      else if constexpr (EPI == W_EPI_MASKY || EPI == W6_EPI_MASKY_Y || EPI == W6_EPI_MASKY_YY) return v6_prefetch_masky(p, cur.R0, cur.n0, wm, wn, lr, lh);
+      else if constexpr (EPI == W_EPI_GY || EPI == W6_EPI_GY_Y) return v6_prefetch_masky<true>(p, cur.R0, cur.n0, wm, wn, lr, lh);
       else return v6_prefetch_c1w(p, cur.R0, cur.n0, wm, wn, lr, lh);
     };
     decltype(prefetch()) pre;
@@ -437,10 +437,17 @@
     } else if constexpr (EPI == W6_EPI_MASKY_Y) {
       if (full) v6_epilogue_masky<true, false, false>(p, acc, pre, nullptr, done.R0, done.n0, wm, wn, lr, lh, done.tm);
       else v6_epilogue_masky<false, false, false>(p, acc, pre, nullptr, done.R0, done.n0, wm, wn, lr, lh, done.tm);
+    } else if constexpr (EPI == W6_EPI_MASKY_YY) {
+      float* xch = reinterpret_cast<float*>(lds + 3 * V6_STAGE);
+      if (full) v6_epilogue_masky<true, false, false, true>(p, acc, pre, xch, done.R0, done.n0, wm, wn, lr, lh, done.tm);
+      else v6_epilogue_masky<false, false, false, true>(p, acc, pre, xch, done.R0, done.n0, wm, wn, lr, lh, done.tm);
     } else if constexpr (EPI == W_EPI_GY) {
       float* xch = reinterpret_cast<float*>(lds + 3 * V6_STAGE);
       if (full) v6_epilogue_masky<true, true>(p, acc, pre, xch, done.R0, done.n0, wm, wn, lr, lh, done.tm);
       else v6_epilogue_masky<false, true>(p, acc, pre, xch, done.R0, done.n0, wm, wn, lr, lh, done.tm);
+    } else if constexpr (EPI == W6_EPI_GY_Y) {
+      if (full) v6_epilogue_masky<true, true, false>(p, acc, pre, nullptr, done.R0, done.n0, wm, wn, lr, lh, done.tm);
+      else v6_epilogue_masky<false, true, false>(p, acc, pre, nullptr, done.R0, done.n0, wm, wn, lr, lh, done.tm);
     } else {
       v6_epilogue_c1w<EPI == W6_EPI_C1W_Y>(p, acc, pre, reinterpret_cast<float*>(lds + 3 * V6_STAGE) + wave * 512, scratch, done.R0,
                                            done.n0, wm, wn, lr, lh, done.tm);
@@ -1191,6 +1198,49 @@
   }
 #pragma unroll
   for (int j = 0; j < 8; ++j) *reinterpret_cast<f32x4*>(v + 16 * j) = o[j];
+}
+
+__global__ __launch_bounds__(256, 4) void wino63_y_fixup_kernel(float* __restrict__ Y, const float* __restrict__ halo,
+                                                              const uint32_t* __restrict__ sbits, const uint32_t* __restrict__ abits,
+                                                              long long hexes, long long tiles, int Tp, int tlim, int C, int ldv,
+                                                              int ld_s, int ld_a, float slope) {
+  const int c4n = C >> 2;
+  const long long idx = (long long)blockIdx.x * blockDim.x + threadIdx.x;
+  if (idx >= (tiles - 1) * c4n) return;
+  const long long t = idx / c4n + 1;
+  const int c = (int)(idx - (t - 1) * c4n) * 4;
+  const long long H = t * V6_BH;
+  if (H >= hexes) return;
+  const int tt = (int)((6 * H) % Tp);
+  if (tt == 0) return;
+  const long long R = 6 * H;
+  const f32x4 c6 = *reinterpret_cast<const f32x4*>(halo + ((t - 1) * 2) * (long long)C + c);
+  const f32x4 c7 = *reinterpret_cast<const f32x4*>(halo + ((t - 1) * 2 + 1) * (long long)C + c);
+  const uint32_t s0 = sbits[R * ld_s + (c >> 5)] >> (c & 31), s1 = sbits[(R + 1) * ld_s + (c >> 5)] >> (c & 31);
+  const uint32_t a0 = abits[R * ld_a + (c >> 5)] >> (c & 31), a1 = abits[(R + 1) * ld_a + (c >> 5)] >> (c & 31);
+  const bool ok0 = tt < tlim, ok1 = tt + 1 < tlim;
+  float* y = Y + v6_at(2 * H, 0, c, ldv >> 3);
+  f32x4 o[7];
+#pragma unroll
+  for (int j = 0; j < 7; ++j) o[j] = *reinterpret_cast<const f32x4*>(y + 16 * j);
+#pragma unroll
+  for (int k = 0; k < 4; ++k) {
+    const float g0 = ok0 ? c6[k] * (((s0 >> k) & 1u) ? 1.f : slope) : 0.f, g1 = ok1 ? c7[k] * (((s1 >> k) & 1u) ? 1.f : slope) : 0.f;
+    const bool odd0 = (a0 >> k) & 1u, odd1 = (a1 >> k) & 1u;
+    const float d0 = odd0 ? 0.f : g0, d1 = odd0 ? g0 : 0.f, d2 = odd1 ? 0.f : g1, d3 = odd1 ? g1 : 0.f;
+    const float ev1 = d0 + d2, od1 = d1 + d3;
+    const float ev2 = fmaf(4.f, d2, d0), od2 = fmaf(8.f, d3, 2.f * d1);
+    const float ev3 = fmaf(0.25f, d2, d0), od3 = fmaf(0.125f, d3, 0.5f * d1);
+    o[0][k] += d0;
+    o[1][k] += ev1 + od1;
+    o[2][k] += ev1 - od1;
+    o[3][k] += ev2 + od2;
+    o[4][k] += ev2 - od2;
+    o[5][k] += ev3 + od3;
+    o[6][k] += ev3 - od3;
+  }
+#pragma unroll
+  for (int j = 0; j < 7; ++j) *reinterpret_cast<f32x4*>(y + 16 * j) = o[j];
 }
 
 __global__ __launch_bounds__(512, 1) void wino63v_tn4y_kernel(const tl_tn_params p, int mtn) {
@@ -1754,12 +1804,24 @@
     TL_REQUIRE(p.auxbits != nullptr, "wino63v_nt: MASK needs auxbits (the sign bits of the stage input)");
     hipLaunchKernelGGL((wino63v_nt_kernel<W_EPI_MASK>), dim3((unsigned)ngrid), dim3(512), 0, st, p);
   } else if (p.epilogue == W_EPI_MASKY) {
-    TL_REQUIRE(p.row_shift == -2 && p.auxbits != nullptr && p.abits != nullptr, "wino63v_nt: epilogue 6 needs row_shift -2, auxbits and abits");
+    TL_REQUIRE((p.row_shift == -2 || p.row_shift == 0) && p.auxbits != nullptr && p.abits != nullptr,
+               "wino63v_nt: epilogue 6 needs row_shift -2 (operand Vd) or 0 (operand Y), auxbits and abits");
     TL_REQUIRE(p.ld_abits * 32 >= p.N && p.Tvalid_in % 2 == 0 && p.Tvalid_in <= 2 * p.Tp, "wino63v_nt: epilogue 6: bad abits / Tvalid_in");
     TL_REQUIRE(p.vout && p.ld_vout >= p.N && p.ld_vout % 8 == 0 && p.vout_quads >= p.M / 3 && p.vout_quads % 2 == 0,
                "wino63v_nt: epilogue 6 needs vout (>= M / 3 hexes, whole pairs, ld_vout %% 8 == 0)");
+    TL_REQUIRE(128LL * 8 * p.ld_vout * 4 < (1LL << 31), "wino63v_nt: ld_vout too large");
+    if (p.row_shift == 0) {
+      TL_REQUIRE(p.vout2 == nullptr && p.vhalo != nullptr, "wino63v_nt: epilogue 6 on a Y operand writes Y only (no vout2) and needs vhalo");
+      TL_REQUIRE(p.ld_auxbits * 32 >= p.N, "wino63v_nt: epilogue 6: ld_auxbits too small");
+      hipLaunchKernelGGL((wino63v_nt_kernel<W6_EPI_MASKY_YY>), dim3((unsigned)ngrid), dim3(512), 0, st, p);
+      if (ntm > 1) {
+        const long long n = (ntm - 1) * (long long)(p.N / 4);
+        hipLaunchKernelGGL(wino63_y_fixup_kernel, dim3((unsigned)((n + 255) / 256)), dim3(256), 0, st, p.vout, p.vhalo, p.auxbits,
+                           p.abits, p.M / 6, ntm, p.Tp, p.Tvalid_in >> 1, p.N, p.ld_vout, p.ld_auxbits, p.ld_abits, p.slope);
+      }
+      return check_launch("wino63v_nt");
+    }
     TL_REQUIRE((p.vout2 == nullptr) == (p.vhalo == nullptr), "wino63v_nt: epilogue 6 takes vout2 and vhalo together (Y and Vd) or neither (Y only)");
-    TL_REQUIRE(128LL * 8 * p.ld_vout * 4 < (1LL << 31), "wino63v_nt: ld_vout too large");
     if (p.vout2 != nullptr) hipLaunchKernelGGL((wino63v_nt_kernel<W_EPI_MASKY>), dim3((unsigned)ngrid), dim3(512), 0, st, p);
     else hipLaunchKernelGGL((wino63v_nt_kernel<W6_EPI_MASKY_Y>), dim3((unsigned)ngrid), dim3(512), 0, st, p);
   } else if (p.epilogue == W_EPI_C1W) {
@@ -1823,11 +1885,13 @@
   TL_REQUIRE(p.auxbits != nullptr && p.abits != nullptr, "conv1_wino63v_dgrad_nt: needs auxbits (sign) and abits (arg-max) of the stage below");
   TL_REQUIRE(p.out_tp > 0 && p.out_tp <= p.Tp && 2 * p.out_tp >= p.Tvalid_in, "conv1_wino63v_dgrad_nt: out_tp = rows per sequence of the bit arrays (0 < out_tp <= Tp, covering Tvalid_in / 2)");
   TL_REQUIRE(p.ld_abits * 32 >= p.N && p.ld_auxbits * 32 >= p.N && p.Tvalid_in % 2 == 0 && p.Tvalid_in <= 2 * p.Tp, "conv1_wino63v_dgrad_nt: bad abits / auxbits / Tvalid_in");
-  TL_REQUIRE(p.vout && p.vout2 && p.vhalo && p.ld_vout >= p.N && p.ld_vout % 8 == 0 && p.vout_quads >= p.M / 3 && p.vout_quads % 2 == 0,
-             "conv1_wino63v_dgrad_nt: needs vout / vout2 (>= M / 3 hexes, whole pairs, ld_vout %% 8 == 0) and vhalo");
+  TL_REQUIRE(p.vout && p.ld_vout >= p.N && p.ld_vout % 8 == 0 && p.vout_quads >= p.M / 3 && p.vout_quads % 2 == 0,
+             "conv1_wino63v_dgrad_nt: needs vout (>= M / 3 hexes, whole pairs, ld_vout %% 8 == 0)");
+  TL_REQUIRE((p.vout2 == nullptr) == (p.vhalo == nullptr), "conv1_wino63v_dgrad_nt: takes vout2 and vhalo together (Y and Vd) or neither (Y only)");
   TL_REQUIRE(128LL * 8 * p.ld_vout * 4 < (1LL << 31), "conv1_wino63v_dgrad_nt: ld_vout too large");
   const long long ngrid = nwg < 256 ? nwg : 256;
-  hipLaunchKernelGGL((wino63v_nt_kernel<W_EPI_GY>), dim3((unsigned)ngrid), dim3(512), 0, (hipStream_t)stream, p);
+  if (p.vout2 != nullptr) hipLaunchKernelGGL((wino63v_nt_kernel<W_EPI_GY>), dim3((unsigned)ngrid), dim3(512), 0, (hipStream_t)stream, p);
+  else hipLaunchKernelGGL((wino63v_nt_kernel<W6_EPI_GY_Y>), dim3((unsigned)ngrid), dim3(512), 0, (hipStream_t)stream, p);
   return check_launch("conv1_wino63v_dgrad_nt");
 }
 
diff --git a/decode_tonal_langauge_amd/csrc/tonal_wino63_epi.h b/decode_tonal_langauge_amd/csrc/tonal_wino63_epi.h
--- a/decode_tonal_langauge_amd/csrc/tonal_wino63_epi.h
+++ b/decode_tonal_langauge_amd/csrc/tonal_wino63_epi.h
@@ -5,7 +5,7 @@
 
 namespace tl {
 
-enum { W6_EPI_MASKY_Y = 8, W6_EPI_C1W_Y = 9, W6_EPI_MASK7 = 10, W6_EPI_MASK7F = 11 };
+enum { W6_EPI_MASKY_Y = 8, W6_EPI_C1W_Y = 9, W6_EPI_MASK7 = 10, W6_EPI_MASK7F = 11, W6_EPI_MASKY_YY = 12, W6_EPI_GY_Y = 13 };
 
 constexpr unsigned V6_DROP = 0x80000000u;
 constexpr unsigned long long V6_HI = 0xffffffff00000000ull;
@@ -299,7 +299,7 @@
 constexpr int v6_stores() {
   return EPI == W_EPI_POOL ? 52 : EPI == W_EPI_POOLV ? 70
          : (EPI == W_EPI_MASK || EPI == W_EPI_LRELU || EPI == W6_EPI_MASK7 || EPI == W6_EPI_MASK7F) ? 96
-         : (EPI == W_EPI_MASKY || EPI == W6_EPI_MASKY_Y || EPI == W_EPI_GY) ? 63 : 0;
+         : (EPI == W_EPI_MASKY || EPI == W6_EPI_MASKY_Y || EPI == W_EPI_GY || EPI == W6_EPI_MASKY_YY || EPI == W6_EPI_GY_Y) ? 63 : 0;
 }
 
 struct v6_pre_mask {
@@ -419,7 +419,7 @@
   }
   return r;
 }
-template <bool FULL, bool DIRECT = false, bool VD = true>
+template <bool FULL, bool DIRECT = false, bool VD = true, bool YOP = false>
 __device__ __forceinline__ void v6_epilogue_masky(const tl_nt_params& p, const f32x16 (&acc)[8], const v6_pre_masky& pre, float* xch,
                                                   long long R0, int n0, int wm, int wn, int lr_in, int lh, long long tm) {
   int lr = lr_in;
@@ -430,8 +430,26 @@
   const long long Rw = R0 + wm * 192;
   const int Tp = p.Tp, hps = Tp / 3;
   const v6_rows rw = v6_rows_of(tm * 128 + wm * 32, Tp);
+  static_assert(!YOP || (!VD && !DIRECT), "the Y-operand form writes Y only and has three taps");
   uint32_t we[3], wo[3], sT[3], firstw = 0;
   (void)hps;
+  uint32_t keepw = ~0u;
+  float c6 = 0.f, c7 = 0.f;
+  if constexpr (YOP) {
+    const int hpsg = Tp / 6;
+    auto starts = [hpsg](int t0) {
+      uint32_t w = 0;
+      for (int e = t0 == 0 ? 0 : hpsg - t0 / 6; e < 16; e += hpsg) w |= 1u << e;
+      return w;
+    };
+    keepw = ~(lh ? starts(rw.tB) : starts(rw.tA));
+    float m[8], d[8];
+#pragma unroll
+    for (int i = 0; i < 8; ++i) m[i] = acc[i][0];
+    wino63_b(m, d);
+    c6 = d[6];
+    c7 = d[7];
+  }
   {
     const bits96 okA = v6_valid_bits96(rw.tA, Tp, p.Tvalid_in >> 1, Rw, p.M);
     const bits96 okB = v6_valid_bits96(rw.tB, Tp, p.Tvalid_in >> 1, Rw + 96, p.M);
@@ -472,9 +490,45 @@
   for (int k = 0; k < 8; ++k) v1keep[k] = 0.f;
   auto andf = [](float x, uint32_t m) { return __uint_as_float(__float_as_uint(x) & m); };
 #pragma unroll
-  for (int e = 0; e < 16; ++e) {
+  for (int it = 0; it < 16; ++it) {
+    const int e = YOP ? ((it + 1) & 15) : it;
     float y[6];
-    if constexpr (DIRECT) {
+    if constexpr (YOP) {
+      if (it == 15) {
+        const int slot = wm * 2 + lh;
+        {
+          float2 v2 = {c6, c7};
+          *reinterpret_cast<float2*>(xch + (slot * 64 + wn * 32 + lr) * 2) = v2;
+        }
+        {
+          const bool hw = wm == 3;
+          const __amdgpu_buffer_rsrc_t rsH = rsrc_of(hw ? p.vhalo + tm * 2 * (long long)p.N : nullptr, hw ? 2LL * p.N * 4 : 0);
+          const unsigned ho = (colok && lh == 1) ? (unsigned)col * 4u : V5_OOB;
+          __builtin_amdgcn_raw_buffer_store_b32(__builtin_bit_cast(unsigned, c6), rsH, ho, 0u, 0);
+          __builtin_amdgcn_raw_buffer_store_b32(__builtin_bit_cast(unsigned, c7), rsH, ho, (unsigned)p.N * 4u, 0);
+        }
+        __builtin_amdgcn_s_waitcnt(0xc07f);
+        __builtin_amdgcn_s_barrier();
+        asm volatile("" ::: "memory");
+        c6 = c7 = 0.f;
+        if (slot > 0) {
+          const float2 v2 = *reinterpret_cast<const float2*>(xch + ((slot - 1) * 64 + wn * 32 + lr) * 2);
+          c6 = v2.x;
+          c7 = v2.y;
+        }
+      }
+      float m[8], d[8];
+#pragma unroll
+      for (int i = 0; i < 8; ++i) m[i] = acc[i][e];
+      wino63_b(m, d);
+      const float kf = __uint_as_float(0x3f800000u & (uint32_t)__builtin_amdgcn_sbfe((int)keepw, e, 1));
+      y[0] = fmaf(c6, kf, d[0]);
+      y[1] = fmaf(c7, kf, d[1]);
+#pragma unroll
+      for (int h = 2; h < 6; ++h) y[h] = d[h];
+      c6 = d[6];
+      c7 = d[7];
+    } else if constexpr (DIRECT) {
 #pragma unroll
       for (int h = 0; h < 6; ++h) y[h] = acc[h][e];
     } else {
```

After: 1294 mel-frames/s (median of 6 runs). About the same (+0.9%).
